# pierluigiferrari/lane_tracker

Hardware: AMD Instinct MI355X
Metric: frames/sec at 1280x720 (end-to-end hot path: undistort+warp+filter_lane_points+sliding_window_search+fit_poly) (higher is better)
Workload: dtype u8; 1 GPU; BASELINE config 3: batch of 256 synthetic lane-like 1280x720 frames per GPU, HBM-resident; warp+filter_lane_points chain + sliding_window_search (26 levels) + fit_poly; bev=1080x1100, parallelism=frames sharded x1, one process per GPU, collective=none (single process), gathered_records_checked=0, streams_per_gpu=4

## Files before the change

include/lane_tracker_amd.h:

```cpp
#ifndef LANE_TRACKER_AMD_H
#define LANE_TRACKER_AMD_H
#include <stddef.h>
#include <stdint.h>

#ifdef __cplusplus
extern "C" {
#endif
#pragma GCC visibility push(default)

#define LT_ABI_VERSION 5

typedef enum lt_status {
    LT_OK = 0,
    LT_ERR_INVALID = -1,
    LT_ERR_HIP = -2,
    LT_ERR_NOMEM = -3,
    LT_ERR_CAPACITY = -4,
    LT_ERR_STATE = -5
} lt_status;

typedef struct lt_ctx lt_ctx;

typedef struct lt_calib {
    int32_t img_w, img_h;
// ... 128 lines not shown

int  lt_bilateral_adaptive_threshold(lt_ctx* ctx, const uint8_t* img, int h, int w, int ksize, int C,
                                     int mode, int true_value, int false_value, uint8_t* out);
int  lt_filter_lane_points(lt_ctx* ctx, const uint8_t* bev_rgb, int h, int w, const lt_filter_params* p,
                           uint8_t* mask);

int  lt_morph_ellipse(lt_ctx* ctx, const uint8_t* img, int h, int w, int k, int op, int direct, uint8_t* out);

int  lt_fit_poly2(lt_ctx* ctx, const int32_t* ys, const int32_t* xs, int n, int h, int w, double coef[3],
                  int* rank_deficient);

int  lt_overlay_configure(lt_ctx* ctx, const double* Minv );
int  lt_overlay_run(lt_ctx* ctx, int first_slot, int n, const int32_t* left_n, const int32_t* right_n,
                    const int32_t* left_yx, const int32_t* right_yx, double alpha);
int  lt_overlay_run_rows(lt_ctx* ctx, int first_slot, int n, const int32_t* left_n, const int32_t* right_n,
                         const int32_t* left_yx, const int32_t* right_yx, double alpha, const int32_t* rows4);
int  lt_overlay_set_font(lt_ctx* ctx, const uint8_t* atlas, const uint8_t* advance, int first_char, int n_glyphs,
                         int glyph_w, int glyph_h);
int  lt_overlay_text(lt_ctx* ctx, int first_slot, int n, const char* lines, int n_lines, int line_len, int x0, int y0,
                     int step);
int  lt_overlay_rows(lt_ctx* ctx, int* row0, int* row1);
int  lt_present_frame(lt_ctx* ctx, int slot, const int32_t* left_n, const int32_t* right_n, const int32_t* left_yx,
                      const int32_t* right_yx, double alpha, const char* lines, int n_lines, int line_len, int x0, int y0,
                      int step, uint8_t* out, const int32_t* rows4);
int  lt_present_lane_async(lt_ctx* ctx, int slot, const int32_t* left_n, const int32_t* right_n, const int32_t* left_yx,
                           const int32_t* right_yx, double alpha, uint8_t* out, const int32_t* rows4);
int  lt_present_finish(lt_ctx* ctx, int slot, const char* lines, int n_lines, int line_len, int x0, int y0, int step,
                       uint8_t* out, const int32_t* rows4);
int  lt_present_lane_from_fit_async(lt_ctx* ctx, int slot, const double* prev_sum, int count, const double* ploty,
                                    const double* ploty2, int n_rows, double alpha, uint8_t* out, const int32_t* rows4);
int  lt_lane_spans_from_fit(lt_ctx* ctx, const double* fit6, int detected, int fit_flags, const double* prev_sum, int count,
                            const double* ploty, const double* ploty2, int n_rows, int16_t* spans_out);
int  lt_lane_polygon_spans(int warp_h, const int32_t* left_yx, int n_left, const int32_t* right_yx, int n_right,
                           int16_t* spans);
int  lt_poly_points(int warp_w, int warp_h, const double* coeffs, int n, const double* ploty, const double* ploty2, int n_rows,
                    int32_t* left_n, int32_t* right_n, int32_t* left_yx, int32_t* right_yx);
int  lt_frame_tail(int warp_w, int warp_h, const double* in, const double* ploty_v, const double* ploty2_v, int n_rows_v, const double* ploty,
                   const double* ploty2, int n_rows, double* avg6, int32_t* left_n, int32_t* right_n, int32_t* left_yx, int32_t* right_yx,
                   double* out);
int  lt_download_overlay(lt_ctx* ctx, int first_slot, int n, uint8_t* out);
int  lt_download_overlay_async(lt_ctx* ctx, int first_slot, int n, uint8_t* out);
int  lt_download_overlay_rows_async(lt_ctx* ctx, int first_slot, int n, uint8_t* out, const int32_t* rows4);
int  lt_download_overlay_wait(lt_ctx* ctx);
int  lt_set_download_method(lt_ctx* ctx, int method);
int  lt_download_stats(lt_ctx* ctx, double* engine_gbs, int* engine_copies, double* kernel_gbs, int* kernel_copies, int* method);
int  lt_overlay_run_strip(lt_ctx* ctx, int first_slot, int n, const int32_t* left_n, const int32_t* right_n, const int32_t* left_yx,
                          const int32_t* right_yx, double alpha);
int  lt_overlay_run_strip_coeffs(lt_ctx* ctx, int first_slot, int n, const double* coeffs, const uint8_t* draw, const double* ploty,
                                 const double* ploty2, int n_rows, double alpha);
int  lt_strip_download_async(lt_ctx* ctx, int first_slot, int n, uint8_t* out, size_t out_frame_stride, int group);
int  lt_text_blend_host(uint8_t* frames, size_t frame_stride, int n, int img_h, int img_w, const uint8_t* atlas, const uint8_t* advance,
                        int first_char, int n_glyphs, int glyph_w, int glyph_h, const char* lines, int n_lines, int line_len, int x0,
                        int y0, int step);
int  lt_host_text_async_group(int group, uint8_t* dst, size_t dst_stride, const uint8_t* src, size_t src_stride, int n, const int32_t* rows4,
                              int img_h, int img_w, const uint8_t* atlas, const uint8_t* advance, int first_char, int n_glyphs,
                              int glyph_w, int glyph_h, const char* lines, int n_lines, int line_len, int x0, int y0, int step);
int  lt_host_text_now_group(int group, uint8_t* frame, int img_h, int img_w, const uint8_t* atlas, const uint8_t* advance, int first_char,
                            int n_glyphs, int glyph_w, int glyph_h, const char* lines, int n_lines, int line_len, int x0, int y0, int step);
int  lt_host_alloc(size_t bytes, void** out);
int  lt_host_copy_async(void* dst, const void* src, size_t bytes);
int  lt_host_copy2d_async(void* dst, size_t dst_pitch, const void* src, size_t src_pitch, size_t width, size_t height);
int  lt_host_copy_wait(void);
int  lt_host_copy_group_create(int* group);
int  lt_host_copy_group_destroy(int group);
int  lt_host_copy_async_group(int group, void* dst, const void* src, size_t bytes);
int  lt_host_copy2d_async_group(int group, void* dst, size_t dst_pitch, const void* src, size_t src_pitch, size_t width, size_t height);
int  lt_host_copy_wait_group(int group);
int  lt_host_touch_async_group(int group, void* p, size_t bytes);
int  lt_shutdown(void);
int  lt_host_copy_stats(double* busy_seconds, double* copied_bytes, long long* pieces, int* threads);
int  lt_host_memory_stats(size_t* staging_bytes, size_t* queued_pieces, size_t* pending_pieces);
int  lt_host_free(void* p);
int  lt_device_cache_trim(size_t keep_bytes);
int  lt_device_cache_stats(size_t* kept_bytes, size_t* live_bytes, size_t* limit_bytes, int* kept_blocks);
int  lt_device_cache_counters(unsigned long long* hits, unsigned long long* misses, unsigned long long* evicted_blocks,
                              unsigned long long* evicted_bytes);
int  lt_download_bev(lt_ctx* ctx, int first_slot, int n, uint8_t* out);

int  lt_calib_source_rows(const lt_calib* calib, int* row0, int* row1);
int  lt_calib_warp_table(const lt_calib* calib, int16_t* xy, uint16_t* frac);
int  lt_calib_undistort_table(const lt_calib* calib, int row0, int row1, int16_t* xy, uint16_t* frac);
int  lt_calib_lab_tables(uint16_t* gamma256, uint16_t* cbrt3072, int32_t* coeffs9);
int  lt_calib_ellipse(int k, int32_t* halfwidths , int* taps);

typedef struct lt_gather lt_gather;
int  lt_gather_init(lt_ctx* ctx, int rank, int world, const char* id_path, int timeout_s, lt_gather** out);
int  lt_gather_world(lt_gather* g, int* rank, int* world);
int  lt_gather_reserve(lt_gather* g, int records_per_rank);
int  lt_gather_stage(lt_gather* g, int first_slot, int n, int at);
int  lt_gather_records(lt_gather* g, int n_records, lt_lane_record* out_host);
int  lt_gather_host(lt_gather* g, const void* in, size_t bytes, void* out);
int  lt_gather_barrier(lt_gather* g);
void lt_gather_destroy(lt_gather* g);

int  lt_timer_start(lt_ctx* ctx);
int  lt_timer_stop(lt_ctx* ctx, float* ms);
int  lt_set_stage_timing(lt_ctx* ctx, int enabled);
int  lt_stage_reset(lt_ctx* ctx);
int  lt_stage_ms(lt_ctx* ctx, float* ms, int32_t* launches, int n);
const char* lt_stage_name(int stage);
#define LT_NO_CONTEXT (-2147483647 - 1)
int  lt_last_threshold_path(lt_ctx* ctx);
int  lt_last_adaptive_path(lt_ctx* ctx);

#pragma GCC visibility pop
#ifdef __cplusplus
}
#endif
#endif
```

lane_tracker_amd/_native.py:

```python
import ctypes as C
import math
import os
import subprocess
import weakref

import numpy as np

_HERE = os.path.dirname(os.path.abspath(__file__))
LIB_PATH = os.environ.get("LANE_TRACKER_AMD_LIB") or os.path.join(_HERE, "liblane_tracker_amd.so")
NUM_STAGES = 12
ABI_VERSION = 5

PLANE_R, PLANE_LAB_B, PLANE_TOPHAT_R, PLANE_TOPHAT_B, PLANE_MERGED, PLANE_MASK = range(6)


class NativeError(RuntimeError):
    pass


class Calib(C.Structure):
    _fields_ = [("img_w", C.c_int32), ("img_h", C.c_int32), ("warp_w", C.c_int32), ("warp_h", C.c_int32),
                ("cam_matrix", C.c_double * 9), ("dist_coeffs", C.c_double * 5), ("M", C.c_double * 9)]


# ... 67 lines not shown
    "lt_download_masks": (C.c_int, [_P, C.c_int, C.c_int, _P]),
    "lt_download_plane": (C.c_int, [_P, C.c_int, C.c_int, C.c_int, _P]),
    "lt_download_undistorted": (C.c_int, [_P, C.c_int, C.c_int, _P]),
    "lt_download_records": (C.c_int, [_P, C.c_int, C.c_int, _P]),
    "lt_download_pixels": (C.c_int, [_P, C.c_int, C.c_int, _P, _P, C.c_int, C.POINTER(C.c_int)]),
    "lt_download_centroids": (C.c_int, [_P, C.c_int, C.c_int, _P, C.c_int, C.POINTER(C.c_int)]),
    "lt_download_lane_lists": (C.c_int, [_P, C.c_int, C.c_void_p, C.c_void_p, C.c_void_p, C.c_void_p, C.c_int, C.POINTER(C.c_int), C.c_int,
                               C.c_void_p, C.c_void_p, C.c_int, C.POINTER(C.c_int)]),
    "lt_copy_records_to_device": (C.c_int, [_P, C.c_int, C.c_int, _P]),
    "lt_enqueue_records_to_device": (C.c_int, [_P, C.c_int, C.c_int, _P]),
    "lt_overlay_configure": (C.c_int, [_P, _P]),
    "lt_overlay_run": (C.c_int, [_P, C.c_int, C.c_int, _P, _P, _P, _P, C.c_double]),
    "lt_overlay_set_font": (C.c_int, [_P, _P, _P, C.c_int, C.c_int, C.c_int, C.c_int]),
    "lt_overlay_text": (C.c_int, [_P, C.c_int, C.c_int, _P, C.c_int, C.c_int, C.c_int, C.c_int, C.c_int]),
    "lt_overlay_rows": (C.c_int, [_P, C.POINTER(C.c_int), C.POINTER(C.c_int)]),
    "lt_present_frame": (C.c_int, [_P, C.c_int, _P, _P, _P, _P, C.c_double, _P, C.c_int, C.c_int, C.c_int, C.c_int, C.c_int, _P, _P]),
    "lt_present_lane_async": (C.c_int, [_P, C.c_int, _P, _P, _P, _P, C.c_double, _P, _P]),
    "lt_present_finish": (C.c_int, [_P, C.c_int, _P, C.c_int, C.c_int, C.c_int, C.c_int, C.c_int, _P, _P]),
    "lt_overlay_run_strip_coeffs": (C.c_int, [_P, C.c_int, C.c_int, _P, _P, _P, _P, C.c_int, C.c_double]),
    "lt_present_lane_from_fit_async": (C.c_int, [_P, C.c_int, _P, C.c_int, _P, _P, C.c_int, C.c_double, _P, _P]),
    "lt_lane_spans_from_fit": (C.c_int, [_P, _P, C.c_int, C.c_int, _P, C.c_int, _P, _P, C.c_int, _P]),
    "lt_lane_polygon_spans": (C.c_int, [C.c_int, _P, C.c_int, _P, C.c_int, _P]),
    "lt_download_overlay": (C.c_int, [_P, C.c_int, C.c_int, _P]),
    "lt_download_overlay_async": (C.c_int, [_P, C.c_int, C.c_int, _P]),
    "lt_download_bev": (C.c_int, [_P, C.c_int, C.c_int, _P]),
    "lt_host_alloc": (C.c_int, [C.c_size_t, C.POINTER(C.c_void_p)]),
    "lt_host_free": (C.c_int, [_P]),
    "lt_host_copy_async": (C.c_int, [_P, _P, C.c_size_t]),
    "lt_host_copy2d_async": (C.c_int, [_P, C.c_size_t, _P, C.c_size_t, C.c_size_t, C.c_size_t]),
    "lt_overlay_run_rows": (C.c_int, [_P, C.c_int, C.c_int, _P, _P, _P, _P, C.c_double, _P]),
    "lt_download_overlay_rows_async": (C.c_int, [_P, C.c_int, C.c_int, _P, _P]),
    "lt_host_copy_wait": (C.c_int, []),
    "lt_host_copy_group_create": (C.c_int, [C.POINTER(C.c_int)]),
    "lt_host_copy_group_destroy": (C.c_int, [C.c_int]),
    "lt_host_copy_async_group": (C.c_int, [C.c_int, _P, _P, C.c_size_t]),
    "lt_host_copy2d_async_group": (C.c_int, [C.c_int, _P, C.c_size_t, _P, C.c_size_t, C.c_size_t, C.c_size_t]),
    "lt_host_copy_wait_group": (C.c_int, [C.c_int]),
    "lt_host_touch_async_group": (C.c_int, [C.c_int, _P, C.c_size_t]),
    "lt_shutdown": (C.c_int, []),
    "lt_host_copy_stats": (C.c_int, [C.POINTER(C.c_double), C.POINTER(C.c_double), C.POINTER(C.c_longlong), C.POINTER(C.c_int)]),
    "lt_warm": (C.c_int, [_P, C.POINTER(SearchParams), C.POINTER(SearchParams), C.c_int]),
    "lt_overlay_run_strip": (C.c_int, [_P, C.c_int, C.c_int, _P, _P, _P, _P, C.c_double]),
    "lt_strip_download_async": (C.c_int, [_P, C.c_int, C.c_int, _P, C.c_size_t, C.c_int]),
    "lt_text_blend_host": (C.c_int, [_P, C.c_size_t, C.c_int, C.c_int, C.c_int, _P, _P, C.c_int, C.c_int, C.c_int, C.c_int, _P, C.c_int,
                                     C.c_int, C.c_int, C.c_int, C.c_int]),
    "lt_host_text_async_group": (C.c_int, [C.c_int, _P, C.c_size_t, _P, C.c_size_t, C.c_int, _P, C.c_int, C.c_int, _P, _P,
                                           C.c_int, C.c_int, C.c_int, C.c_int, _P, C.c_int, C.c_int, C.c_int, C.c_int, C.c_int]),
    "lt_host_text_now_group": (C.c_int, [C.c_int, _P, C.c_int, C.c_int, _P, _P, C.c_int, C.c_int, C.c_int, C.c_int, _P, C.c_int, C.c_int,
                                         C.c_int, C.c_int, C.c_int]),
    "lt_mask_run": (C.c_int, [_P, C.c_int, C.c_int, C.POINTER(FilterParams)]),
    "lt_mask_rerun": (C.c_int, [_P, C.c_int, C.c_int, C.POINTER(FilterParams)]),
    "lt_upload_bev": (C.c_int, [_P, _P, C.c_int, C.c_int]),
    "lt_filter_run": (C.c_int, [_P, C.c_int, C.c_int, C.POINTER(FilterParams)]),
    "lt_sws_fit_run": (C.c_int, [_P, C.c_int, C.c_int, C.POINTER(SearchParams)]),
    "lt_band_fit_run": (C.c_int, [_P, C.c_int, C.c_int, C.POINTER(SearchParams), _P]),
    "lt_search_fit_list": (C.c_int, [_P, C.c_int, _P, C.POINTER(SearchParams), C.POINTER(SearchParams)]),
    "lt_upload_frame_rows_list": (C.c_int, [_P, _P, C.c_int, C.c_int]),
    "lt_upload_frame_rest_list": (C.c_int, [_P, _P, C.c_int, C.c_int]),
    "lt_band_fit_chain_run": (C.c_int, [_P, C.c_int, C.c_int, C.POINTER(SearchParams), _P]),
    "lt_band_fit_chain_collect": (C.c_int, [_P, C.c_int, C.c_int, _P]),
    "lt_band_fit_chain_cancel": (C.c_int, [_P]),
    "lt_set_search_cus": (C.c_int, [_P, C.c_int]),
    "lt_set_walk_min_frames": (C.c_int, [_P, C.c_int]),
    "lt_set_direct_upload": (C.c_int, [_P, C.c_int]),
    "lt_direct_upload_count": (C.c_ulonglong, [_P]),
    "lt_set_urgent": (C.c_int, [_P, C.c_int]),
    "lt_poly_points": (C.c_int, [C.c_int, C.c_int, _P, C.c_int, _P, _P, C.c_int, _P, _P, _P, _P]),
    "lt_frame_tail": (C.c_int, [C.c_int, C.c_int, _P, _P, _P, C.c_int, _P, _P, C.c_int, _P, _P, _P, _P, _P, _P]),
    "lt_download_overlay_wait": (C.c_int, [_P]),
    "lt_set_frame_base": (C.c_int, [_P, C.c_int, C.c_int, C.c_int]),
    "lt_mask_batch": (C.c_int, [_P, _P, C.c_int, C.POINTER(FilterParams), _P]),
    "lt_sws_fit_batch": (C.c_int, [_P, _P, C.c_int, C.POINTER(SearchParams), _P]),
    "lt_band_fit_batch": (C.c_int, [_P, _P, C.c_int, C.POINTER(SearchParams), _P, _P]),
    "lt_bilateral_adaptive_threshold": (C.c_int, [_P, _P, C.c_int, C.c_int, C.c_int, C.c_int, C.c_int, C.c_int,
                                                 C.c_int, _P]),
    "lt_filter_lane_points": (C.c_int, [_P, _P, C.c_int, C.c_int, C.POINTER(FilterParams), _P]),
    "lt_morph_ellipse": (C.c_int, [_P, _P, C.c_int, C.c_int, C.c_int, C.c_int, C.c_int, _P]),
    "lt_fit_poly2": (C.c_int, [_P, _P, _P, C.c_int, C.c_int, C.c_int, C.POINTER(C.c_double), C.POINTER(C.c_int)]),
    "lt_calib_source_rows": (C.c_int, [C.POINTER(Calib), C.POINTER(C.c_int), C.POINTER(C.c_int)]),
    "lt_calib_warp_table": (C.c_int, [C.POINTER(Calib), _P, _P]),
    "lt_calib_undistort_table": (C.c_int, [C.POINTER(Calib), C.c_int, C.c_int, _P, _P]),
    "lt_calib_lab_tables": (C.c_int, [_P, _P, _P]),
    "lt_calib_ellipse": (C.c_int, [C.c_int, _P, C.POINTER(C.c_int)]),
    "lt_gather_init": (C.c_int, [_P, C.c_int, C.c_int, C.c_char_p, C.c_int, C.POINTER(_P)]),
    "lt_gather_world": (C.c_int, [_P, C.POINTER(C.c_int), C.POINTER(C.c_int)]),
    "lt_gather_reserve": (C.c_int, [_P, C.c_int]),
    "lt_gather_stage": (C.c_int, [_P, C.c_int, C.c_int, C.c_int]),
    "lt_gather_records": (C.c_int, [_P, C.c_int, _P]),
    "lt_gather_host": (C.c_int, [_P, _P, C.c_size_t, _P]),
    "lt_gather_barrier": (C.c_int, [_P]),
    "lt_gather_destroy": (None, [_P]),
    "lt_timer_start": (C.c_int, [_P]),
    "lt_timer_stop": (C.c_int, [_P, C.POINTER(C.c_float)]),
    "lt_set_stage_timing": (C.c_int, [_P, C.c_int]),
    "lt_stage_reset": (C.c_int, [_P]),
    "lt_stage_ms": (C.c_int, [_P, C.POINTER(C.c_float), C.POINTER(C.c_int32), C.c_int]),
    "lt_stage_name": (C.c_char_p, [C.c_int]),
    "lt_device_cache_trim": (C.c_int, [C.c_size_t]),
    "lt_device_cache_stats": (C.c_int, [C.POINTER(C.c_size_t), C.POINTER(C.c_size_t), C.POINTER(C.c_size_t), C.POINTER(C.c_int)]),
    "lt_device_cache_counters": (C.c_int, [C.POINTER(C.c_ulonglong)] * 4),
    "lt_host_memory_stats": (C.c_int, [C.POINTER(C.c_size_t)] * 3),
    "lt_set_download_method": (C.c_int, [_P, C.c_int]),
    "lt_download_stats": (C.c_int, [_P, _P, _P, _P, _P, _P]),
    "lt_last_threshold_path": (C.c_int, [_P]),
    "lt_last_adaptive_path": (C.c_int, [_P]),
    "lt_set_input_format": (C.c_int, [_P, C.c_int, _P]),
    "lt_get_input_format": (C.c_int, [_P, C.POINTER(C.c_int), _P]),
    "lt_yuv_to_rgb": (C.c_int, [_P, _P, C.c_int, C.c_int, C.c_int, _P, _P]),
    "lt_attach_device_frames": (C.c_int, [_P, _P, C.c_int, C.c_int]),
    "lt_device_frames_rest": (C.c_int, [_P, C.c_int, C.c_int, _P]),
    "lt_device_alloc": (C.c_int, [C.c_int, C.c_size_t, C.POINTER(C.c_void_p)]),
    "lt_device_free": (C.c_int, [_P]),
    "lt_device_write": (C.c_int, [_P, _P, C.c_size_t]),
    "lt_device_read": (C.c_int, [_P, _P, C.c_size_t]),
    "lt_device_stream_wait": (C.c_int, [C.c_int, C.c_size_t]),
}

PIXEL_FORMATS = {"rgb": 0, "nv12": 1, "i420": 2}
YUV_MATRICES = {"bt601": (1220542, 1673527, -852492, -409993, 2116026),
                "bt709": (1220542, 1880097, -558891, -223347, 2214593)}


def pixel_format_id(pixel_format):
    try:
        return PIXEL_FORMATS[pixel_format]
    except (KeyError, TypeError):
        raise ValueError("pixel_format must be 'rgb', 'nv12' or 'i420', got %r" % (pixel_format,)) from None


def yuv_coeffs(matrix):
    if isinstance(matrix, str):
        if matrix not in YUV_MATRICES:
            raise ValueError("yuv_matrix must be 'bt601' or 'bt709', got %r" % (matrix,))
        matrix = YUV_MATRICES[matrix]
    k = np.ascontiguousarray(matrix, dtype=np.int32)
    if k.shape != (5,):
        raise ValueError("a conversion matrix is five integers")
    return k


def frame_shape(img_size, pixel_format="rgb"):
    w, h = int(img_size[0]), int(img_size[1])
    if pixel_format_id(pixel_format) == 0:
        return (h, w, 3)
    if w % 2 or h % 2:
        raise ValueError("4:2:0 frames need an even width and height, got %dx%d" % (w, h))
    return (h * 3 // 2, w)

_lib = None


def build(force=False):
    csrc = os.path.join(_HERE, "csrc")
    cmd = ["make", "-C", csrc, "-s", "-j8"] + (["-B"] if force else [])
    subprocess.check_call(cmd)
    return LIB_PATH


def load():
    global _lib
    if _lib is not None:
        return _lib
    if not os.path.exists(LIB_PATH):
        raise NativeError(f"{LIB_PATH} is missing: build it with `python -c 'import __graft_entry__ as g; g.build()'` "
                          "(hipcc --offload-arch=gfx950).  lane_tracker_amd has no CPU fallback.")
    lib = C.CDLL(LIB_PATH)
# ... 196 lines not shown
    if rc:
        _check(rc)


def host_copy_stats():
    b, y, p, t = C.c_double(), C.c_double(), C.c_longlong(), C.c_int()
    _check(load().lt_host_copy_stats(C.byref(b), C.byref(y), C.byref(p), C.byref(t)))
    return {"busy_s": b.value, "bytes": y.value, "pieces": p.value, "threads": t.value}


def device_cache_stats():
    k, l, m, n = C.c_size_t(), C.c_size_t(), C.c_size_t(), C.c_int()
    _check(load().lt_device_cache_stats(C.byref(k), C.byref(l), C.byref(m), C.byref(n)))
    return {"kept_bytes": k.value, "live_bytes": l.value, "limit_bytes": m.value, "kept_blocks": n.value}


def host_memory_stats():
    v = [C.c_size_t() for _ in range(3)]
    _check(load().lt_host_memory_stats(*[C.byref(x) for x in v]))
    return dict(zip(("staging_bytes", "queued_pieces", "pending_pieces"), (int(x.value) for x in v)))


def device_cache_counters():
    v = [C.c_ulonglong() for _ in range(4)]
    _check(load().lt_device_cache_counters(*[C.byref(x) for x in v]))
    return dict(zip(("hits", "misses", "evicted_blocks", "evicted_bytes"), (int(x.value) for x in v)))


def pinned_empty(shape, dtype=np.uint8):
    return _pinned.empty(shape, dtype)


def _u8(a, shape_tail=None):
    a = np.ascontiguousarray(a, dtype=np.uint8)
    return a


def filter_params(filter_type="bilateral", ksize_r=15, C_r=8, ksize_b=35, C_b=5, mask_noise=False,
                  noise_thresh=140, ksize_noise=65, C_noise=10):
    ft = {"bilateral": 0, "neighborhood": 1}.get(filter_type, 2)
    return FilterParams(ft, int(ksize_r), int(C_r), int(ksize_b), int(C_b), int(bool(mask_noise)),
                        int(noise_thresh), int(ksize_noise), int(C_noise))


def search_params(window_width=30, window_height=40, search_range=20, mu=0.1, no_success_limit=8,
                  start_slice=0.25, ignore_sides=360, ignore_bottom=30, bandwidth=25, partial=1.0):
    return SearchParams(int(window_width), int(window_height), int(search_range), int(no_success_limit),
                        int(ignore_sides), int(ignore_bottom), int(bandwidth), 0, float(mu), float(start_slice),
                        float(partial))


def make_calib(img_size, warped_size, cam_matrix, dist_coeffs, M):
    cal = Calib()
    cal.img_w, cal.img_h = int(img_size[0]), int(img_size[1])
    cal.warp_w, cal.warp_h = int(warped_size[0]), int(warped_size[1])
    cal.cam_matrix[:] = [float(v) for v in np.asarray(cam_matrix, np.float64).reshape(9)]
    d = np.asarray(dist_coeffs, np.float64).reshape(-1)
    cal.dist_coeffs[:] = [float(v) for v in (list(d[:5]) + [0.0] * 5)[:5]]
    cal.M[:] = [float(v) for v in np.asarray(M, np.float64).reshape(9)]
    return cal


def calib_tables(cal):
    lib = load()
    r0, r1 = C.c_int(0), C.c_int(0)
    _check(lib.lt_calib_source_rows(C.byref(cal), C.byref(r0), C.byref(r1)))
    wxy = np.empty((cal.warp_h, cal.warp_w, 2), np.int16)
    wfr = np.empty((cal.warp_h, cal.warp_w), np.uint16)
    _check(lib.lt_calib_warp_table(C.byref(cal), wxy.ctypes.data, wfr.ctypes.data))
    uxy = np.empty((r1.value - r0.value, cal.img_w, 2), np.int16)
    ufr = np.empty((r1.value - r0.value, cal.img_w), np.uint16)
    _check(lib.lt_calib_undistort_table(C.byref(cal), r0.value, r1.value, uxy.ctypes.data, ufr.ctypes.data))
    gamma, cbrt, coef = np.empty(256, np.uint16), np.empty(3072, np.uint16), np.empty(9, np.int32)
    _check(lib.lt_calib_lab_tables(gamma.ctypes.data, cbrt.ctypes.data, coef.ctypes.data))
    ell = {}
    for k in (5, 29, 55):
        dx, taps = np.empty(k, np.int32), C.c_int(0)
        _check(lib.lt_calib_ellipse(k, dx.ctypes.data, C.byref(taps)))
        ell[k] = (dx, taps.value)
    return dict(source_rows=(r0.value, r1.value), warp_xy=wxy, warp_frac=wfr, und_xy=uxy, und_frac=ufr, gamma=gamma,
                cbrt=cbrt, lab_coeffs=coef, ellipse=ell)


def pack_polygons(polygons):
    ln = np.array([len(p[0]) for p in polygons], np.int32)
    rn = np.array([len(p[2]) for p in polygons], np.int32)

    def pairs(ys, xs, counts):
        out = np.empty((int(counts.sum()), 2), np.int32)
        at = 0
        for y, x, m in zip(ys, xs, counts):
            out[at:at + m, 0] = y
            out[at:at + m, 1] = x
            at += m
        return out
    return ln, rn, pairs([p[0] for p in polygons], [p[1] for p in polygons], ln), pairs([p[2] for p in polygons], [p[3] for p in polygons], rn)


def poly_points(warped_size, coeffs, ploty, ploty2):
    lib = load()
    coeffs = np.ascontiguousarray(coeffs, np.float64).reshape(-1, 6)
    ploty, ploty2 = np.ascontiguousarray(ploty, np.float64), np.ascontiguousarray(ploty2, np.float64)
    n, rows = coeffs.shape[0], ploty.shape[0]
    ln, rn = np.empty(n, np.int32), np.empty(n, np.int32)
    lyx, ryx = np.empty((n * rows, 2), np.int32), np.empty((n * rows, 2), np.int32)
    _check(lib.lt_poly_points(int(warped_size[0]), int(warped_size[1]), coeffs.ctypes.data, n, ploty.ctypes.data, ploty2.ctypes.data,
                              rows, ln.ctypes.data, rn.ctypes.data, lyx.ctypes.data, ryx.ctypes.data))
    return ln, rn, lyx[:int(ln.sum())], ryx[:int(rn.sum())]


class Context:

    def __init__(self, img_size, warped_size, cam_matrix, dist_coeffs, M, device=0, capacity=1):
        self._h = None
        lib = load()
        cal = make_calib(img_size, warped_size, cam_matrix, dist_coeffs, M)
        h = _P()
        _check(lib.lt_create(C.byref(cal), int(device), C.byref(h)))
        self._h = h
        self.lib = lib
        self.img_w, self.img_h, self.warp_w, self.warp_h = cal.img_w, cal.img_h, cal.warp_w, cal.warp_h
        self._frame_tail = (cal.img_h, cal.img_w, 3)
        self.reserve(capacity)

    def close(self):
        if self._h is not None:
            self.lib.lt_destroy(self._h)
            self._h = None

    def __del__(self):
        try:
            self.close()
        except Exception:
            pass

    def reserve(self, capacity):
        _check(self.lib.lt_reserve(self._h, int(capacity)))
        self.capacity = max(getattr(self, "capacity", 0), int(capacity))

    def info(self):
        i = Info()
        _check(self.lib.lt_get_info(self._h, C.byref(i)))
        return i

    def sync(self):
        _check(self.lib.lt_sync(self._h))

    def set_streams(self, n):
        _check(self.lib.lt_set_streams(self._h, int(n)))

    def set_input_format(self, pixel_format="rgb", yuv_matrix="bt601"):
        layout = pixel_format_id(pixel_format)
        tail = frame_shape((self.img_w, self.img_h), pixel_format)
        k = yuv_coeffs(yuv_matrix) if layout else None
        _check(self.lib.lt_set_input_format(self._h, layout, None if k is None else k.ctypes.data))
        self._frame_tail = tail

    def input_format(self):
        layout, k = C.c_int(0), np.zeros(5, np.int32)
        _check(self.lib.lt_get_input_format(self._h, C.byref(layout), k.ctypes.data))
        return {v: n for n, v in PIXEL_FORMATS.items()}[layout.value], tuple(int(v) for v in k)

    def _frames(self, frames):
        f = _u8(frames)
        tail = self._frame_tail
        if f.shape[-len(tail):] != tail or f.ndim > len(tail) + 1:
# ... 496 lines not shown
```

lane_tracker_amd/csrc/k_tophat.hip:

```cpp
#include <cstdlib>

#include <cstdio>
#include <cstdlib>

#include <type_traits>

#include "lt_internal.h"

#ifndef LT_DPP_SELECT
#define LT_DPP_SELECT 0
#endif
#ifndef LT_FUSED55
#define LT_FUSED55 1
#endif

namespace lt {
namespace {

typedef unsigned short u16x2 __attribute__((ext_vector_type(2)));

template <bool DIL>
__device__ __forceinline__ uint32_t pk(uint32_t a, uint32_t b) {
    const u16x2 x = __builtin_bit_cast(u16x2, a), y = __builtin_bit_cast(u16x2, b);
    const u16x2 r = DIL ? __builtin_elementwise_max(x, y) : __builtin_elementwise_min(x, y);
// ... 16 lines not shown
    static constexpr int slot_width[17] = {0, 7, 10, 12, 14, 16, 17, 18, 19, 20, 21, 22, 23, 24, 25, 26, 27};
    static constexpr int slot(int j) { return half_slot[j <= R ? j : K - 1 - j]; }

    template <bool DIL>
    static __device__ __forceinline__ void row_windows(uint32_t* s, int lane, uint32_t (&H)[NH]) {
        uint32_t* S0 = s + MARGIN;
        uint32_t* S1 = S0 + PLANE;
        uint32_t* S2 = S0 + 2 * PLANE;
        uint32_t* S4 = S0 + 3 * PLANE;
        uint32_t* S7 = S0 + 4 * PLANE;
        uint32_t* S14 = S0 + 5 * PLANE;
        const int pa = lane, pb = lane + 64;
        S1[pa] = pk<DIL>(pk<DIL>(S0[pa - 1], S0[pa + 1]), S0[pa]);
        S1[pb] = pk<DIL>(pk<DIL>(S0[pb - 1], S0[pb + 1]), S0[pb]);
        wave_lds_fence();
        S2[pa] = pk<DIL>(S1[pa - 1], S1[pa + 1]);
        S2[pb] = pk<DIL>(S1[pb - 1], S1[pb + 1]);
        wave_lds_fence();
        S4[pa] = pk<DIL>(S2[pa - 2], S2[pa + 2]);
        S4[pb] = pk<DIL>(S2[pb - 2], S2[pb + 2]);
        wave_lds_fence();
        S7[pa] = pk<DIL>(S4[pa - 3], S4[pa + 3]);
        S7[pb] = pk<DIL>(S4[pb - 3], S4[pb + 3]);
        wave_lds_fence();
        S14[pa] = pk<DIL>(S7[pa - 7], S7[pa + 7]);
        S14[pb] = pk<DIL>(S7[pb - 7], S7[pb + 7]);
        wave_lds_fence();
        const int p = R + lane;
        H[0] = S0[p];
        H[1] = S7[p];
        H[2] = pk<DIL>(S7[p - 3], S7[p + 3]);
        H[3] = pk<DIL>(S7[p - 5], S7[p + 5]);
        H[4] = S14[p];
#pragma unroll
        for (int t = 2; t <= 13; ++t) H[3 + t] = pk<DIL>(S14[p - t], S14[p + t]);
    }
};

struct SE29 {
    static constexpr int K = 29, R = 14, NH = 9, NPLANES = 5;
    static constexpr int half_slot[15] = {0, 1, 2, 3, 4, 5, 5, 6, 7, 7, 7, 8, 8, 8, 8};
    static constexpr int slot_width[9] = {0, 5, 7, 9, 10, 11, 12, 13, 14};
    static constexpr int slot(int j) { return half_slot[j <= R ? j : K - 1 - j]; }

    template <bool DIL>
    static __device__ __forceinline__ void row_windows(uint32_t* s, int lane, uint32_t (&H)[NH]) {
        uint32_t* S0 = s + MARGIN;
        uint32_t* S1 = S0 + PLANE;
        uint32_t* S2 = S0 + 2 * PLANE;
        uint32_t* S4 = S0 + 3 * PLANE;
        uint32_t* S7 = S0 + 4 * PLANE;
        const int pa = lane, pb = lane + 64;
        S1[pa] = pk<DIL>(pk<DIL>(S0[pa - 1], S0[pa + 1]), S0[pa]);
        S1[pb] = pk<DIL>(pk<DIL>(S0[pb - 1], S0[pb + 1]), S0[pb]);
        wave_lds_fence();
        S2[pa] = pk<DIL>(S1[pa - 1], S1[pa + 1]);
        S2[pb] = pk<DIL>(S1[pb - 1], S1[pb + 1]);
        wave_lds_fence();
        S4[pa] = pk<DIL>(S2[pa - 2], S2[pa + 2]);
        S4[pb] = pk<DIL>(S2[pb - 2], S2[pb + 2]);
        wave_lds_fence();
        S7[pa] = pk<DIL>(S4[pa - 3], S4[pa + 3]);
        S7[pb] = pk<DIL>(S4[pb - 3], S4[pb + 3]);
        wave_lds_fence();
        const int p = R + lane;
        H[0] = S0[p];
        H[1] = pk<DIL>(S4[p - 1], S4[p + 1]);
        H[2] = S7[p];
#pragma unroll
        for (int t = 2; t <= 7; ++t) H[1 + t] = pk<DIL>(S7[p - t], S7[p + t]);
    }
};

struct RunsGeom {
    int h, w, nstrips, nbands, band_rows, ntasks;
    size_t plane_stride;
    int dpitch;
    size_t dst_stride;
    int nframes;
    int nstrips_normal;
    int n_normal;
    int xcd;
    uint8_t* copy_dst;
};

struct LaneCols {
    uint32_t off[4];
    uint32_t keep[2];
    uint32_t fill[2];
};

__device__ __forceinline__ LaneCols lane_cols(int col0, int w, bool second, uint32_t n8) {
    LaneCols c;
#pragma unroll
    for (int e = 0; e < 2; ++e) {
        const int ca = col0 + 64 * e, cb = ca + 64;
        const bool va = ca >= 0 && ca < w && (e == 0 || second), vb = cb >= 0 && cb < w && (e == 0 || second);
        c.off[2 * e] = (uint32_t)min(max(ca, 0), w - 1);
        c.off[2 * e + 1] = (uint32_t)min(max(cb, 0), w - 1);
        c.keep[e] = (va ? 0xffffu : 0u) | (vb ? 0xffff0000u : 0u);
        c.fill[e] = (va ? 0u : n8) | (vb ? 0u : (n8 << 16));
    }
    return c;
}

__device__ __forceinline__ uint32_t fetch_entry(const uint8_t* __restrict__ row, const LaneCols& c, int e) {
    const uint32_t a = row[c.off[2 * e]], b = row[c.off[2 * e + 1]];
    return ((a | (b << 16)) & c.keep[e]) | c.fill[e];
}

__device__ __forceinline__ uint32_t fetch_entry(__amdgpu_buffer_rsrc_t plane, int row_off, const LaneCols& c, int e) {
    const uint32_t a = __builtin_amdgcn_raw_buffer_load_b8(plane, (int)c.off[2 * e], row_off, 0);
    const uint32_t b = __builtin_amdgcn_raw_buffer_load_b8(plane, (int)c.off[2 * e + 1], row_off, 0);
    return ((a | (b << 16)) & c.keep[e]) | c.fill[e];
}

template <class SE, bool DIL>
__global__ __launch_bounds__(256) void k_morph_runs(const uint8_t* __restrict__ src, uint8_t* __restrict__ dst,
                                                   const uint8_t* __restrict__ minuend, RunsGeom g) {
    __shared__ uint32_t s_chain[4][SE::NPLANES * PLANE];
    constexpr int K = SE::K, R = SE::R, NH = SE::NH;
    constexpr uint32_t NEUTRAL = DIL ? 0u : 0x00ff00ffu;
    const int lane = threadIdx.x & 63, wv = threadIdx.x >> 6;
    const int task = __builtin_amdgcn_readfirstlane(blockIdx.x * 4 + wv);
    if (task >= g.ntasks) return;
    const int strip = task % g.nstrips;
    const int band = (task / g.nstrips) % g.nbands;
    const int frame = task / (g.nstrips * g.nbands);
    const uint8_t* s = src + (size_t)frame * g.plane_stride;
    uint8_t* d = dst + (size_t)frame * g.dst_stride;
    const uint8_t* m = minuend ? minuend + (size_t)frame * g.plane_stride : nullptr;
    uint32_t* chain = s_chain[wv];
    const int x0 = strip * 128;
    const int yb0 = band * g.band_rows, yb1 = min(yb0 + g.band_rows, g.h);
    const int xa = x0 + lane, xb = xa + 64;
    const bool va = xa < g.w, vb = xb < g.w;
    const int oa = min(xa, g.w - 1), ob = min(xb, g.w - 1);

    uint32_t A[K];
#pragma unroll
    for (int j = 0; j < K; ++j) A[j] = NEUTRAL;

    const int y_first = yb0 - R, y_last = yb1 - 1 + R;
    const LaneCols cols = lane_cols(x0 - R + lane, g.w, lane + 64 < 64 + 2 * R, NEUTRAL & 0xffu);
    const uint8_t* row = s + (size_t)min(max(y_first, 0), g.h - 1) * g.w;
    uint32_t e0 = fetch_entry(row, cols, 0), e1 = fetch_entry(row, cols, 1);
    uint32_t ma = 0, mb = 0;
    for (int yy = y_first; yy <= y_last; ++yy) {
        const bool in_img = yy >= 0 && yy < g.h;
        chain[MARGIN + lane] = in_img ? e0 : NEUTRAL;
        chain[MARGIN + lane + 64] = in_img ? e1 : NEUTRAL;
        wave_lds_fence();
        row = s + (size_t)min(max(yy + 1, 0), g.h - 1) * g.w;
        e0 = fetch_entry(row, cols, 0);
        e1 = fetch_entry(row, cols, 1);
        const int y = yy - R;
        const uint32_t ma_cur = ma, mb_cur = mb;
        if (m) {
            const uint8_t* mrow = m + (size_t)min(max(y + 1, 0), g.h - 1) * g.w;
            ma = mrow[oa];
            mb = mrow[ob];
        }

        uint32_t H[NH];
        SE::template row_windows<DIL>(chain, lane, H);
        wave_lds_fence();
// ... 188 lines not shown
            updates(std::integral_constant<int, 4>{});
        }
        asm volatile("s_waitcnt lgkmcnt(0)" : "+v"(a5), "+v"(b5), "+v"(c5), "+v"(d5), "+v"(e5) :: "memory");
        {
            LT_PAIR(15, a5, b5)
            Ha[16] = op3<DIL>(lo(c5), lo(d5), lo(e5)); Hb[16] = op3<DIL>(hi(c5), hi(d5), hi(e5));
            updates(std::integral_constant<int, 5>{});
        }
#undef LT_WAIT8
#undef LT_PAIR
#undef LT_G
#pragma unroll
        for (int j = 0; j < K; ++j) A[j] = An[j];
        out_ab[1] = A[0];
    } else if (SE::K == 55) {
        LT_STEP3(2, 3, 9)
        const uint32_t a4 = lds_addr(S4 + p - 8), a13 = lds_addr(SL + p - 14);
        unsigned long long r0, f[7], g[29];
        LT_RD64(r0, s0_rd, 0);
        LT_RD64(f[0], a4, 0);
        LT_RD64(f[1], a4, 16);
        LT_RD64(f[2], a4, 40);
        LT_RD64(f[3], a4, 64);
        LT_RD64(f[4], a4, 88);
        LT_RD64(f[5], a4, 112);
        LT_RD64(f[6], a4, 128);
#define LT_G(i) LT_RD64(g[i], a13, (i) * 8)
        LT_G(0); LT_G(1); LT_G(2); LT_G(3); LT_G(4); LT_G(5); LT_G(6); LT_G(7); LT_G(8); LT_G(9); LT_G(10); LT_G(11);
        LT_G(13); LT_G(14); LT_G(15);
        LT_G(17); LT_G(18); LT_G(19); LT_G(20); LT_G(21); LT_G(22); LT_G(23); LT_G(24); LT_G(25); LT_G(26); LT_G(27); LT_G(28);
#undef LT_G
        asm volatile("s_waitcnt lgkmcnt(0)"
                     : "+v"(r0), "+v"(f[0]), "+v"(f[1]), "+v"(f[2]), "+v"(f[3]), "+v"(f[4]), "+v"(f[5]), "+v"(f[6]),
                       "+v"(g[0]), "+v"(g[1]), "+v"(g[2]), "+v"(g[3]), "+v"(g[4]), "+v"(g[5]), "+v"(g[6]), "+v"(g[7]),
                       "+v"(g[8]), "+v"(g[9]), "+v"(g[10]), "+v"(g[11]), "+v"(g[13]), "+v"(g[14]), "+v"(g[15])
                     :: "memory");
        asm volatile("" : "+v"(g[17]), "+v"(g[18]), "+v"(g[19]), "+v"(g[20]), "+v"(g[21]), "+v"(g[22]), "+v"(g[23]),
                          "+v"(g[24]), "+v"(g[25]), "+v"(g[26]), "+v"(g[27]), "+v"(g[28]) :: "memory");
        __builtin_amdgcn_sched_barrier(0);
        Ha[0] = lo(r0); Hb[0] = hi(r0);
        Ha[1] = op2<DIL>(lo(f[2]), lo(f[4])); Hb[1] = op2<DIL>(hi(f[2]), hi(f[4]));
        Ha[2] = op3<DIL>(lo(f[1]), lo(f[3]), lo(f[5])); Hb[2] = op3<DIL>(hi(f[1]), hi(f[3]), hi(f[5]));
        Ha[3] = op3<DIL>(lo(f[0]), lo(f[3]), lo(f[6])); Hb[3] = op3<DIL>(hi(f[0]), hi(f[3]), hi(f[6]));
        Ha[4] = op2<DIL>(lo(g[13]), lo(g[15])); Hb[4] = op2<DIL>(hi(g[13]), hi(g[15]));
#pragma unroll
        for (int q = 3; q <= 13; ++q) {
            Ha[2 + q] = op2<DIL>(lo(g[14 - q]), lo(g[14 + q]));
            Hb[2 + q] = op2<DIL>(hi(g[14 - q]), hi(g[14 + q]));
        }
        Ha[16] = op3<DIL>(lo(g[0]), lo(g[14]), lo(g[28])); Hb[16] = op3<DIL>(hi(g[0]), hi(g[14]), hi(g[28]));
    } else {
        const uint32_t a4 = lds_addr(S4 + p - 10);
        unsigned long long r0, g[21];
        LT_PRIO_READS2();
        LT_RD64(r0, s0_rd, 0);
#define LT_G(i) LT_RD64(g[i], a4, (i) * 8)
        LT_G(9); LT_G(11); LT_G(7); LT_G(13); LT_G(10); LT_G(5); LT_G(15); LT_G(4); LT_G(16); LT_G(3); LT_G(17); LT_G(2); LT_G(18);
        LT_G(1); LT_G(19); LT_G(0); LT_G(20);
#undef LT_G
        LT_PRIO_MATH2();
        asm volatile("s_waitcnt lgkmcnt(10)" : "+v"(r0), "+v"(g[9]), "+v"(g[11]), "+v"(g[7]), "+v"(g[13]), "+v"(g[10]), "+v"(g[5]), "+v"(g[15]) :: "memory");
        Ha[0] = lo(r0); Hb[0] = hi(r0);
        Ha[1] = op2<DIL>(lo(g[9]), lo(g[11])); Hb[1] = op2<DIL>(hi(g[9]), hi(g[11]));
        Ha[2] = op2<DIL>(lo(g[7]), lo(g[13])); Hb[2] = op2<DIL>(hi(g[7]), hi(g[13]));
        Ha[3] = op3<DIL>(lo(g[5]), lo(g[10]), lo(g[15])); Hb[3] = op3<DIL>(hi(g[5]), hi(g[10]), hi(g[15]));
        asm volatile("" : "+v"(Ha[0]), "+v"(Hb[0]), "+v"(Ha[1]), "+v"(Hb[1]), "+v"(Ha[2]), "+v"(Hb[2]), "+v"(Ha[3]), "+v"(Hb[3]));
        asm volatile("s_waitcnt lgkmcnt(0)"
                     : "+v"(g[0]), "+v"(g[1]), "+v"(g[2]), "+v"(g[3]), "+v"(g[4]), "+v"(g[16]), "+v"(g[17]), "+v"(g[18]), "+v"(g[19]), "+v"(g[20])
                     :: "memory");
#pragma unroll
        for (int t = 6; t <= 9; ++t) {
            Ha[t - 2] = op3<DIL>(lo(g[10 - t]), lo(g[10]), lo(g[10 + t]));
            Hb[t - 2] = op3<DIL>(hi(g[10 - t]), hi(g[10]), hi(g[10 + t]));
        }
        Ha[8] = op3<DIL>(Ha[2], lo(g[0]), lo(g[20])); Hb[8] = op3<DIL>(Hb[2], hi(g[0]), hi(g[20]));

    }
#undef LT_STEP3
#undef LT_RD64
}

template <class SE, bool DIL, bool WIDE, bool TH, bool PAIR, bool COPYM = false>
__device__ __forceinline__ void morph_task(const uint8_t* __restrict__ src, uint8_t* __restrict__ dst, const uint8_t* __restrict__ minuend,
                                           const RunsGeom& g, uint2* chain, uint8_t* s_out_w, int lane, int strip, int band, int frame) {
    static_assert(WIDE || !PAIR, "pair strips exist for the WIDE kernels only");
    static_assert(!COPYM || (WIDE && TH), "the minuend copy rides on the dword store of the WIDE top-hat");
    constexpr int K = SE::K, R = SE::R, NH = SE::NH;
    constexpr uint32_t NEUTRAL = (DIL ? 0u : 0x00ff00ffu) | BIAS2;
    const uint8_t* s = src + (size_t)frame * g.plane_stride;
    uint8_t* d = dst + (size_t)frame * g.dst_stride;
    const uint8_t* m = TH ? minuend + (size_t)frame * g.plane_stride : nullptr;
    const bool has_b = PAIR && frame + 1 < g.nframes;
    const bool lane_b = PAIR && (lane & 16);
    const int x0 = strip * 128;
    const int yb0 = band * g.band_rows, yb1 = min(yb0 + g.band_rows, g.h);
    const int xa = x0 + lane, xb = xa + 64;
    const bool va = xa < g.w, vb = xb < g.w;
    const int oa = min(xa, g.w - 1), ob = min(xb, g.w - 1);

    const int wcol = x0 + 4 * (lane & (PAIR ? 15 : 31)), wcol_c = min(wcol, g.w - 4);
    const uint32_t row_sel = lane < 32 ? 0x06040200u : 0x07050301u;

    uint32_t A[K];
#pragma unroll
    for (int j = 0; j < K; ++j) A[j] = NEUTRAL;

    const int y_first = yb0 - R, y_last = yb1 - 1 + R;
    const int c0 = x0 - R + lane;
    const uint32_t col_a = (uint32_t)min(max(c0, 0), g.w - 1), col_b = (uint32_t)min(max(c0 + 64, 0), g.w - 1), col_c = (uint32_t)min(max(c0 + 128, 0), g.w - 1);
    constexpr int RSRC_RAW = 0x00027000;
    const int plane_bytes = g.h * g.w;
    const int b_src = has_b ? (int)g.plane_stride : 0;
    const __amdgpu_buffer_rsrc_t src_rs = __builtin_amdgcn_make_buffer_rsrc(const_cast<uint8_t*>(s), 0, plane_bytes + b_src, RSRC_RAW);
    const __amdgpu_buffer_rsrc_t dst_rs = __builtin_amdgcn_make_buffer_rsrc(d + (size_t)yb0 * g.dpitch, 0, (yb1 - yb0) * g.dpitch + (has_b ? (int)g.dst_stride : 0), RSRC_RAW);
    const __amdgpu_buffer_rsrc_t min_rs = __builtin_amdgcn_make_buffer_rsrc(const_cast<uint8_t*>(TH ? m : s), 0, plane_bytes + b_src, RSRC_RAW);
    const __amdgpu_buffer_rsrc_t cp_rs = __builtin_amdgcn_make_buffer_rsrc(
        (COPYM ? g.copy_dst + (size_t)frame * g.dst_stride : d) + (size_t)yb0 * g.dpitch, 0, (yb1 - yb0) * g.dpitch + (has_b ? (int)g.dst_stride : 0), RSRC_RAW);
    auto row_ptr = [&](int y) { return __mul24(min(max(y, 0), g.h - 1), g.w); };
    struct Raw { uint32_t a, b, c, d; };
    const uint32_t sel_ab = 0x0c000c00u | ((4u + (col_b & 3u)) << 16) | (col_a & 3u);
    const uint32_t sel_bc = 0x0c000c00u | ((4u + (col_c & 3u)) << 16) | (col_b & 3u);
    const uint32_t sel_pa = 0x0c000c00u | ((4u + (col_a & 3u)) << 16) | (col_a & 3u);
    const uint32_t sel_pb = 0x0c000c00u | ((4u + (col_b & 3u)) << 16) | (col_b & 3u);
    auto load_row = [&](int y) __attribute__((always_inline)) {
        const int ro = row_ptr(y);
        Raw r;
        r.d = 0;
        if (PAIR) {
            r.a = __builtin_amdgcn_raw_buffer_load_b32(src_rs, (int)(col_a & ~3u), ro, 0);
            r.b = __builtin_amdgcn_raw_buffer_load_b32(src_rs, (int)(col_b & ~3u), ro, 0);
            r.c = __builtin_amdgcn_raw_buffer_load_b32(src_rs, (int)(col_a & ~3u), ro + b_src, 0);
            r.d = __builtin_amdgcn_raw_buffer_load_b32(src_rs, (int)(col_b & ~3u), ro + b_src, 0);
        } else if (WIDE) {
            r.a = __builtin_amdgcn_raw_buffer_load_b32(src_rs, (int)(col_a & ~3u), ro, 0);
            r.b = __builtin_amdgcn_raw_buffer_load_b32(src_rs, (int)(col_b & ~3u), ro, 0);
            r.c = __builtin_amdgcn_raw_buffer_load_b32(src_rs, (int)(col_c & ~3u), ro, 0);
        } else {
            r.a = __builtin_amdgcn_raw_buffer_load_b8(src_rs, (int)col_a, ro, 0);
            r.b = __builtin_amdgcn_raw_buffer_load_b8(src_rs, (int)col_b, ro, 0);
            r.c = __builtin_amdgcn_raw_buffer_load_b8(src_rs, (int)col_c, ro, 0);
        }
        return r;
    };
    auto combine = [&](const Raw& r, uint32_t& e0, uint32_t& e1) __attribute__((always_inline)) {
        if (PAIR) {
            asm volatile("v_perm_b32 %0, %4, %2, %6\n\tv_perm_b32 %1, %5, %3, %7" : "=&v"(e0), "=&v"(e1) : "v"(r.a), "v"(r.b), "v"(r.c), "v"(r.d), "v"(sel_pa), "v"(sel_pb));
        } else if (WIDE) {
            asm volatile("v_perm_b32 %0, %3, %2, %5\n\tv_perm_b32 %1, %4, %3, %6" : "=&v"(e0), "=&v"(e1) : "v"(r.a), "v"(r.b), "v"(r.c), "v"(sel_ab), "v"(sel_bc));
        } else {
            e0 = r.a | (r.b << 16);
            e1 = r.b | (r.c << 16);
            asm volatile("" : "+v"(e0), "+v"(e1));
        }
        if (LT_MORPH_BIAS) { e0 |= BIAS2; e1 |= BIAS2; }
    };
    uint32_t ea0, ea1, eb0, eb1;
    combine(load_row(y_first), ea0, ea1);
    combine(load_row(y_first + 1), eb0, eb1);
    uint32_t ma0 = 0, mb0 = 0, ma1 = 0, mb1 = 0;
    uint32_t m_off = (uint32_t)(__mul24(yb0 - 2 * R + (lane >> 5), g.w) + wcol_c + (lane_b ? b_src : 0));
    uint32_t st_off = wcol < g.w && (!lane_b || has_b) ? (uint32_t)(__mul24(-2 * R - 2 + (lane >> 5), g.dpitch) + wcol + (lane_b ? (int)g.dst_stride : 0))
                                                      : 0x80000000u;
    uint32_t mcur = 0;
    const uint32_t s0_rd = (uint32_t)(uintptr_t)(chain + MARGIN + ((R + lane) & 63));
    const uint32_t out_wr = (uint32_t)(uintptr_t)(s_out_w + (WIDE ? 2 * lane : 0));
    const uint32_t out_rd = (uint32_t)(uintptr_t)(s_out_w + (WIDE ? 8 * (lane & 31) : 0));
    auto out_issue = [&](unsigned long long& q) { asm volatile("ds_read_b64 %0, %1" : "=v"(q) : "v"(out_rd) : "memory"); };
    auto out_finish = [&](unsigned long long q, uint32_t mp, int yp) {
        asm volatile("s_waitcnt lgkmcnt(0)" : "+v"(q) :: "memory");
        uint32_t v = __builtin_amdgcn_perm((uint32_t)(q >> 32), (uint32_t)q, row_sel);
        if (TH) v = mp - v;
        if (PAIR) {
            const int row = yp + (lane >> 5);
            if (row >= yb0 && row < yb1) {
                __builtin_amdgcn_raw_buffer_store_b32(v, dst_rs, (int)st_off, 0, 0);
                if (COPYM) __builtin_amdgcn_raw_buffer_store_b32(mp, cp_rs, (int)st_off, 0, 0);
            }
        } else {
            __builtin_amdgcn_raw_buffer_store_b32(v, dst_rs, (int)st_off, 0, 0);
            if (COPYM) __builtin_amdgcn_raw_buffer_store_b32(mp, cp_rs, (int)st_off, 0, 0);
        }
    };
    auto row_pair = [&](int yy) __attribute__((always_inline)) {
        const uint2 e_pa = make_uint2(ea0, eb0);
        const uint2 e_pb = make_uint2(ea1, eb1);
        chain[MARGIN + lane] = lane < R ? e_pb : e_pa;
        wave_lds_fence();
        const Raw ra = load_row(yy + 2), rb = load_row(yy + 3);
        const int y = yy - R;
        const uint32_t ca0 = ma0, cb0 = mb0, ca1 = ma1, cb1 = mb1;
        const uint32_t mprev = mcur;
        if (TH) {
            if (WIDE) {
                mcur = __builtin_amdgcn_raw_buffer_load_b32(min_rs, (int)m_off, 0, 0);
            } else {
                const uint8_t* r0 = m + (size_t)min(max(y + 2, 0), g.h - 1) * g.w;
                const uint8_t* r1 = m + (size_t)min(max(y + 3, 0), g.h - 1) * g.w;
                ma0 = r0[oa]; mb0 = r0[ob];
                ma1 = r1[oa]; mb1 = r1[ob];
            }
        }
        uint32_t Ha[NH], Hb[NH];
        constexpr bool FUSE = LT_FUSED55 && K == 55;
        uint32_t out_ab[2];
        row_windows2<SE, DIL, FUSE>(chain, lane, e_pa, e_pb, s0_rd, Ha, Hb, A, out_ab);
        wave_lds_fence();
        const bool prev_out = WIDE && y - 1 >= yb0 && y - 2 < yb1;
        unsigned long long q = 0;
        if (prev_out) out_issue(q);
        if (WIDE) __builtin_amdgcn_sched_barrier(0);
        if (!FUSE) {
            out_ab[0] = op2<DIL>(A[1], Ha[SE::slot(0)]);
#pragma unroll
            for (int j = 0; j < K - 2; ++j) A[j] = op3<DIL>(A[j + 2], Ha[SE::slot(j + 1)], Hb[SE::slot(j)]);
            A[K - 2] = op2<DIL>(Ha[SE::slot(K - 1)], Hb[SE::slot(K - 2)]);
            A[K - 1] = Hb[SE::slot(K - 1)];
            out_ab[1] = A[0];
        }
        const uint32_t out_a = out_ab[0], out_b = out_ab[1];
        if (WIDE) {
            __builtin_amdgcn_sched_barrier(0);
            out_finish(q, mprev, y - 2);
            if (y + 1 >= yb0 && y < yb1) {
                const uint32_t W = __builtin_amdgcn_perm(out_b, out_a, 0x06020400u);
                asm volatile("ds_write_b16 %0, %1\n\tds_write_b16_d16_hi %0, %1 offset:128" :: "v"(out_wr), "v"(W) : "memory");
            }
            m_off += 2u * (uint32_t)g.w;
            st_off += 2u * (uint32_t)g.dpitch;
        } else
#pragma unroll
        for (int rr = 0; rr < 2; ++rr) {
            const int yo = y + rr;
            if (yo >= yb0 && yo < yb1) {
                const uint32_t o2 = rr == 0 ? out_a : out_b;
                uint32_t oa_v = o2 & 0xffu, ob_v = (o2 >> 16) & 0xffu;
                if (TH) {
                    const uint32_t qa = rr == 0 ? ca0 : ca1, qb = rr == 0 ? cb0 : cb1;
                    oa_v = qa - oa_v;
                    ob_v = qb - ob_v;
                }
                const size_t o = (size_t)yo * g.dpitch;
                if (va) d[o + xa] = (uint8_t)oa_v;
                if (vb) d[o + xb] = (uint8_t)ob_v;
            }
        }
        combine(ra, ea0, ea1);
        combine(rb, eb0, eb1);
    };
    constexpr int PAIRS = (LT_FUSED55 && K == 55) ? 2 : 1;
    for (int yy = y_first; yy <= y_last; yy += 2 * PAIRS) {
        row_pair(yy);
        if (PAIRS == 2) row_pair(yy + 2);
    }
    if (WIDE) {
        const int npairs = (y_last - y_first) / 2 + 1, pairs_run = (npairs + PAIRS - 1) / PAIRS * PAIRS;
        const int y_tail = y_first + 2 * (pairs_run - 1) - R;
        unsigned long long q;
        out_issue(q);
        out_finish(q, mcur, y_tail);
    }
}

#ifndef LT_MORPH_WPB
#define LT_MORPH_WPB 4
#endif
#ifdef LT_MORPH_MAX_WAVES
#define LT_MORPH_WAVES_ATTR __attribute__((amdgpu_waves_per_eu(1, LT_MORPH_MAX_WAVES)))
#else
#define LT_MORPH_WAVES_ATTR
#endif
template <class SE, bool DIL, bool WIDE, bool TH, bool COPYM = false>
__global__ __launch_bounds__(64 * LT_MORPH_WPB) LT_MORPH_WAVES_ATTR void k_morph_runs2(const uint8_t* __restrict__ src, uint8_t* __restrict__ dst,
                                                    const uint8_t* __restrict__ minuend, RunsGeom g) {
    __shared__ uint2 s_chain[LT_MORPH_WPB][4 * PLANE];
    __shared__ __attribute__((aligned(8))) uint8_t s_out[WIDE ? LT_MORPH_WPB : 1][WIDE ? 256 : 8];
    const int lane = threadIdx.x & 63, wv = threadIdx.x >> 6;
    uint32_t bid = blockIdx.x;
    if (g.xcd) {
        const uint32_t total = gridDim.x, q = total >> 3, r = total & 7u, xcd = bid & 7u, k = bid >> 3;
        bid = (xcd < r ? xcd * (q + 1) : r * (q + 1) + (xcd - r) * q) + k;
    }
    const int task = __builtin_amdgcn_readfirstlane((int)bid * LT_MORPH_WPB + wv);
    if (task >= g.ntasks) return;
    if (!LT_MORPH_BIAS) __builtin_amdgcn_s_setreg(1 | (6 << 6) | (1 << 11), 3);
    const int n_pair = g.ntasks - g.n_normal;
    if (!WIDE || task >= n_pair) {
        const int t = task - n_pair;
        const int strip = t % g.nstrips_normal;
        const int band = (t / g.nstrips_normal) % g.nbands;
        const int frame = t / (g.nstrips_normal * g.nbands);
        morph_task<SE, DIL, WIDE, TH, false, COPYM>(src, dst, minuend, g, s_chain[wv], s_out[wv], lane, strip, band, frame);
    } else if constexpr (WIDE) {
        morph_task<SE, DIL, WIDE, TH, true, COPYM>(src, dst, minuend, g, s_chain[wv], s_out[wv], lane, g.nstrips_normal, task % g.nbands, 2 * (task / g.nbands));
    }
}

template <class SE, bool DIL, bool TH, int Q>
__device__ __forceinline__ void morph_one_task(const int task, const uint8_t* __restrict__ src, uint8_t* __restrict__ dst,
                                               const uint8_t* __restrict__ minuend, const RunsGeom& g, uint2 (*s_chain)[4 * PLANE],
                                               uint32_t (*s_ring)[3 * 2 * Q][64]) {
    constexpr int K = SE::K, R = SE::R, NH = SE::NH, S = 2 * Q, RING = 3 * S;
    static_assert(S - 1 <= K - 1, "the pipeline must be longer than a step");
    const int lane = threadIdx.x & 63, wv = __builtin_amdgcn_readfirstlane((int)(threadIdx.x >> 6));
    if (!LT_MORPH_BIAS) __builtin_amdgcn_s_setreg(1 | (6 << 6) | (1 << 11), 3);
    const int strip = task % g.nstrips;
    const int band = (task / g.nstrips) % g.nbands;
    const int frame = task / (g.nstrips * g.nbands);
    const uint8_t* s = src + (size_t)frame * g.plane_stride;
    uint8_t* d = dst + (size_t)frame * g.dst_stride;
    const uint8_t* m = TH ? minuend + (size_t)frame * g.plane_stride : nullptr;
    uint2* chain = s_chain[wv];
    const int x0 = strip * 128;
    const int yb0 = band * g.band_rows, yb1 = min(yb0 + g.band_rows, g.h);
    const int xa = x0 + lane, xb = xa + 64;
    const bool va = xa < g.w, vb = xb < g.w;
    const int oa = min(xa, g.w - 1), ob = min(xb, g.w - 1);
    const int y_first = yb0 - R, y_base = yb0 - 2 * R;
    const int npairs = (yb1 - yb0 + 2 * R + 1) / 2, nsteps = (npairs + Q - 1) / Q;
    const int c0 = x0 - R + lane;
    const uint32_t col_a = (uint32_t)min(max(c0, 0), g.w - 1), col_b = (uint32_t)min(max(c0 + 64, 0), g.w - 1), col_c = (uint32_t)min(max(c0 + 128, 0), g.w - 1);
    constexpr int RSRC_RAW = 0x00027000;
    const __amdgpu_buffer_rsrc_t src_rs = __builtin_amdgcn_make_buffer_rsrc(const_cast<uint8_t*>(s), 0, g.h * g.w, RSRC_RAW);
    auto row_off = [&](int y) { return __mul24(min(max(y, 0), g.h - 1), g.w); };
    const uint32_t sel_ab = 0x0c000c00u | ((4u + (col_b & 3u)) << 16) | (col_a & 3u);
    const uint32_t sel_bc = 0x0c000c00u | ((4u + (col_c & 3u)) << 16) | (col_b & 3u);
    struct Raw { uint32_t a, b, c; };
    auto load_row = [&](int y) __attribute__((always_inline)) {
        const int ro = row_off(y);
        Raw r;
        r.a = __builtin_amdgcn_raw_buffer_load_b32(src_rs, (int)(col_a & ~3u), ro, 0);
        r.b = __builtin_amdgcn_raw_buffer_load_b32(src_rs, (int)(col_b & ~3u), ro, 0);
        r.c = __builtin_amdgcn_raw_buffer_load_b32(src_rs, (int)(col_c & ~3u), ro, 0);
        return r;
    };
    auto combine = [&](const Raw& r, uint32_t& e0, uint32_t& e1) __attribute__((always_inline)) {
        asm volatile("v_perm_b32 %0, %3, %2, %5\n\tv_perm_b32 %1, %4, %3, %6" : "=&v"(e0), "=&v"(e1) : "v"(r.a), "v"(r.b), "v"(r.c), "v"(sel_ab), "v"(sel_bc));
        if (LT_MORPH_BIAS) { e0 |= BIAS2; e1 |= BIAS2; }
    };
    constexpr uint32_t NEUTRAL = (DIL ? 0u : 0x00ff00ffu) | BIAS2;
    uint32_t A[K + 1];
#pragma unroll
    for (int p = 0; p <= K; ++p) A[p] = NEUTRAL;
    uint32_t ea0, ea1, eb0, eb1;
    {
        const int yy = y_first + 2 * wv;
        combine(load_row(yy), ea0, ea1);
        combine(load_row(yy + 1), eb0, eb1);
    }
    const uint32_t s0_rd = (uint32_t)(uintptr_t)(chain + MARGIN + ((R + lane) & 63));
    for (int t = 0; t < nsteps; ++t) {
        const int yy = y_first + 2 * (t * Q + wv);
        const uint2 e_pa = make_uint2(ea0, eb0);
        const uint2 e_pb = make_uint2(ea1, eb1);
        chain[MARGIN + lane] = lane < R ? e_pb : e_pa;
        wave_lds_fence();
        const Raw ra = load_row(yy + S), rb = load_row(yy + S + 1);
        const int o0 = S * t + 2 * wv, yo = y_base + o0;
        uint32_t m0a = 0, m0b = 0, m1a = 0, m1b = 0;
        if (TH) {
            const uint8_t* r0 = m + (size_t)min(max(yo, 0), g.h - 1) * g.w;
            const uint8_t* r1 = m + (size_t)min(max(yo + 1, 0), g.h - 1) * g.w;
            m0a = r0[oa]; m0b = r0[ob];
            m1a = r1[oa]; m1b = r1[ob];
        }
        uint32_t Ha[NH], Hb[NH];
        row_windows2<SE, DIL, false>(chain, lane, e_pa, e_pb, s0_rd, Ha, Hb);
        wave_lds_fence();
        uint32_t An[K + 1];
#pragma unroll
        for (int p = 0; p <= K; ++p) {
            const int j = p - 1;
            const bool prev = j + S <= K - 1, ha = j <= K - 2, hb = j >= 0;
            const uint32_t va_ = Ha[SE::slot(j + 1 <= K - 1 ? j + 1 : K - 1)], vb_ = Hb[SE::slot(j >= 0 ? j : 0)];
            const uint32_t vp = A[prev ? p + S : K];
            An[p] = prev && ha && hb ? op3<DIL>(vp, va_, vb_) : prev && ha ? op2<DIL>(vp, va_) : ha && hb ? op2<DIL>(va_, vb_) : vb_;
        }
// ... 8 lines not shown
#pragma unroll
        for (int p = S; p <= K; ++p) A[p] = An[p];
        __syncthreads();
        {
            const int sl0 = o0 % RING, sl1 = sl0 + 1 == RING ? 0 : sl0 + 1;
            uint32_t v0 = s_ring[0][sl0][lane], v1 = s_ring[0][sl1][lane];
#pragma unroll
            for (int q = 1; q < Q; ++q) {
                v0 = op2<DIL>(v0, s_ring[q][sl0][lane]);
                v1 = op2<DIL>(v1, s_ring[q][sl1][lane]);
            }
#pragma unroll
            for (int rr = 0; rr < 2; ++rr) {
                const int y = yo + rr;
                if (y >= yb0 && y < yb1) {
                    const uint32_t v = rr == 0 ? v0 : v1;
                    uint32_t pa = v & 0xffu, pb = (v >> 16) & 0xffu;
                    if (TH) {
                        pa = (rr == 0 ? m0a : m1a) - pa;
                        pb = (rr == 0 ? m0b : m1b) - pb;
                    }
                    const size_t o = (size_t)y * g.dpitch;
                    if (va) d[o + xa] = (uint8_t)pa;
                    if (vb) d[o + xb] = (uint8_t)pb;
                }
            }
        }
        combine(ra, ea0, ea1);
        combine(rb, eb0, eb1);
    }
}

template <class SE, bool DIL, bool TH, int Q>
__global__ __launch_bounds__(64 * Q) void k_morph_one(const uint8_t* __restrict__ src, uint8_t* __restrict__ dst,
                                                      const uint8_t* __restrict__ minuend, RunsGeom g) {
    __shared__ uint2 s_chain[Q][4 * PLANE];
    __shared__ uint32_t s_ring[Q][3 * 2 * Q][64];
    morph_one_task<SE, DIL, TH, Q>((int)blockIdx.x, src, dst, minuend, g, s_chain, s_ring);
}

template <bool DIL, bool TH, int Q>
__global__ __launch_bounds__(64 * Q) void k_morph_one_pair(const uint8_t* __restrict__ src55, uint8_t* __restrict__ dst55, const uint8_t* __restrict__ min55, RunsGeom g55,
                                                           const uint8_t* __restrict__ src29, uint8_t* __restrict__ dst29, const uint8_t* __restrict__ min29, RunsGeom g29) {
    __shared__ uint2 s_chain[Q][4 * PLANE];
    __shared__ uint32_t s_ring[Q][3 * 2 * Q][64];
    const int task = (int)blockIdx.x;
    if (task < g55.ntasks) morph_one_task<SE55, DIL, TH, Q>(task, src55, dst55, min55, g55, s_chain, s_ring);
    else morph_one_task<SE29, DIL, TH, Q>(task - g55.ntasks, src29, dst29, min29, g29, s_chain, s_ring);
}

template <class SE, int Q>
void launch_one(hipStream_t s, const uint8_t* src, uint8_t* dst, const uint8_t* minuend, bool dilate, const RunsGeom& g) {
    const dim3 grid(g.ntasks), block(64 * Q);
    if (dilate && minuend) hipLaunchKernelGGL((k_morph_one<SE, true, true, Q>), grid, block, 0, s, src, dst, minuend, g);
    else if (dilate) hipLaunchKernelGGL((k_morph_one<SE, true, false, Q>), grid, block, 0, s, src, dst, minuend, g);
    else hipLaunchKernelGGL((k_morph_one<SE, false, false, Q>), grid, block, 0, s, src, dst, minuend, g);
}

static void one_frame_bands(RunsGeom& g, int n, int want_wgs) {
    int cus1 = 256, dev1 = 0;
    (void)hipGetDevice(&dev1);
    (void)hipDeviceGetAttribute(&cus1, hipDeviceAttributeMultiprocessorCount, dev1);
    const int target = want_wgs > 0 ? want_wgs : 2 * cus1;
    int nb = std::max(1, target / std::max(1, n * g.nstrips));
    int rows = std::max((g.h + nb - 1) / nb, 8);
    rows = (rows + 1) & ~1;
    g.band_rows = rows;
    g.nbands = (g.h + rows - 1) / rows;
    g.nstrips_normal = g.nstrips;
    g.ntasks = g.n_normal = n * g.nstrips * g.nbands;
    g.xcd = 0;
}

template <class SE>
bool table_matches(const EllipseSE& se) {
    if (se.k != SE::K) return false;
    for (int j = 0; j < SE::K; ++j)
        if (SE::slot_width[SE::slot(j)] != se.dx[j]) return false;
    return true;
}

template <class SE>
bool launch_runs(hipStream_t s, const uint8_t* src, uint8_t* dst, const uint8_t* minuend, int h, int w, bool dilate,
                 size_t plane_stride, int n, int dpitch, size_t dst_stride, uint8_t* copy_dst) {
    RunsGeom g;
    g.copy_dst = copy_dst;
    g.h = h;
    g.w = w;
    g.plane_stride = plane_stride;
    g.dpitch = dpitch > 0 ? dpitch : w;
    g.dst_stride = dpitch > 0 ? dst_stride : plane_stride;
    g.nstrips = (w + 127) / 128;
    g.nframes = n;
    static const bool one_row = [] { const char* e = LT_EXP_ENV("LT_MORPH_ONE_ROW"); return e && e[0] == '1'; }();
    static const bool narrow = [] { const char* e = LT_EXP_ENV("LT_MORPH_WIDE"); return e && e[0] == '0'; }();
    const bool wide = !narrow && (w & 3) == 0 && (plane_stride & 3) == 0 && w >= 4 && (g.dpitch & 3) == 0 && (g.dst_stride & 3) == 0 &&
                      ((uintptr_t)dst & 3) == 0 && ((uintptr_t)minuend & 3) == 0;
    static const int one_q = [] { const char* e = LT_EXP_ENV("LT_MORPH_ONE"); return e ? std::atoi(e) : 4; }();
    if (n <= 2 && (one_q == 4 || one_q == 8) && !one_row && wide && !copy_dst && ((uintptr_t)src & 3) == 0) {
        static const int want_wgs = [] { const char* e = LT_EXP_ENV("LT_MORPH_ONE_WGS"); return e ? std::atoi(e) : 0; }();
        one_frame_bands(g, n, want_wgs);
        if (one_q == 8) launch_one<SE, 8>(s, src, dst, minuend, dilate, g);
        else launch_one<SE, 4>(s, src, dst, minuend, dilate, g);
        return true;
    }
    int dev = 0, cus = 256, blocks_per_cu = 3;
    (void)hipGetDevice(&dev);
    (void)hipDeviceGetAttribute(&cus, hipDeviceAttributeMultiprocessorCount, dev);
    {
        const void* fn = one_row ? (dilate ? (const void*)k_morph_runs<SE, true> : (const void*)k_morph_runs<SE, false>)
                                 : wide ? (dilate ? (minuend ? (const void*)k_morph_runs2<SE, true, true, true> : (const void*)k_morph_runs2<SE, true, true, false>)
                                                  : (const void*)k_morph_runs2<SE, false, true, false>)
                                        : (dilate ? (minuend ? (const void*)k_morph_runs2<SE, true, false, true> : (const void*)k_morph_runs2<SE, true, false, false>)
                                                  : (const void*)k_morph_runs2<SE, false, false, false>);
        int nb = 0;
        const int threads = one_row ? 256 : 64 * LT_MORPH_WPB;
        if (hipOccupancyMaxActiveBlocksPerMultiprocessor(&nb, fn, threads, 0) == hipSuccess && nb > 0) blocks_per_cu = nb * threads / 256;
        if (blocks_per_cu < 1) blocks_per_cu = 1;
    }
    const long long slots = (long long)cus * blocks_per_cu * 4, simds = (long long)cus * 4;
    int best_nb = 1;
    double best_cost = 1e300;
    for (int nb = 1; nb <= 256; ++nb) {
        const int rows = (h + nb - 1) / nb;
        const int real_nb = (h + rows - 1) / rows;
        const long long tasks = (long long)n * g.nstrips * real_nb;
        if (nb > 1 && rows < (tasks <= simds ? 4 : tasks <= slots ? (SE::R + 1) / 2 : 2 * SE::R)) break;
        const double rounds = (double)((tasks + slots - 1) / slots);
        const double cost = tasks <= simds ? (double)(rows + 2 * SE::R) : tasks < slots ? 1.15 * (rows + 2 * SE::R) : rounds * (rows + 2 * SE::R);
        if (cost < best_cost - 1e-9) { best_cost = cost; best_nb = nb; }
    }
    if ((long long)n * g.nstrips * 4 >= slots && h / 4 >= 2 * SE::R) best_nb = 4;
    else if ((long long)n * g.nstrips * 4 >= slots / 4 && h / 4 >= 2 * SE::R) best_nb = 4;
#ifdef LT_EXPERIMENTS
    {
        char name[32];
        std::snprintf(name, sizeof name, "LT_MORPH_NB_%d%c", SE::K, dilate ? 'D' : 'E');
        const char* e = std::getenv(name);
        if (e && std::atoi(e) > 0) best_nb = std::atoi(e);
    }
#endif
    g.band_rows = (h + best_nb - 1) / best_nb;
    g.nbands = (h + g.band_rows - 1) / g.band_rows;
    static const bool no_pair = [] { const char* e = LT_EXP_ENV("LT_MORPH_PAIR"); return e && e[0] == '0'; }();
    const bool pair_strip = wide && !one_row && !no_pair && w - 128 * (g.nstrips - 1) <= 64 &&
                            (long long)plane_stride + (long long)h * w < (1ll << 31) && (long long)g.dst_stride + (long long)h * g.dpitch < (1ll << 31);
    g.nstrips_normal = pair_strip ? g.nstrips - 1 : g.nstrips;
    g.n_normal = n * g.nstrips_normal * g.nbands;
    g.ntasks = g.n_normal + (pair_strip ? (n + 1) / 2 * g.nbands : 0);
    static const bool want_xcd = [] { const char* e = LT_EXP_ENV("LT_MORPH_XCD"); return e && e[0] == '1'; }();
    g.xcd = want_xcd ? 1 : 0;
    dim3 grid((g.ntasks + 3) / 4);
    const dim3 grid2((g.ntasks + LT_MORPH_WPB - 1) / LT_MORPH_WPB), block2(64 * LT_MORPH_WPB);
    if (copy_dst && one_row) return false;
    if (one_row) {
        if (dilate) hipLaunchKernelGGL((k_morph_runs<SE, true>), grid, dim3(256), 0, s, src, dst, minuend, g);
        else hipLaunchKernelGGL((k_morph_runs<SE, false>), grid, dim3(256), 0, s, src, dst, minuend, g);
    } else {
        static const int extra_lds = [] { const char* e = LT_EXP_ENV("LT_MORPH_EXTRA_LDS"); return e ? std::atoi(e) : 0; }();
        const bool th = dilate && minuend != nullptr;
        if (copy_dst) {
            if constexpr (SE::K == 55) {
                if (!wide || !th || ((uintptr_t)copy_dst & 3)) return false;
                hipLaunchKernelGGL((k_morph_runs2<SE, true, true, true, true>), grid2, block2, extra_lds, s, src, dst, minuend, g);
                return true;
            } else
                return false;
        }
#define LT_LAUNCH(DIL_, WIDE_, TH_) hipLaunchKernelGGL((k_morph_runs2<SE, DIL_, WIDE_, TH_>), grid2, block2, extra_lds, s, src, dst, minuend, g)
        if (wide) {
            if (th) LT_LAUNCH(true, true, true);
            else if (dilate) LT_LAUNCH(true, true, false);
            else LT_LAUNCH(false, true, false);
        } else {
            if (th) LT_LAUNCH(true, false, true);
            else if (dilate) LT_LAUNCH(true, false, false);
            else LT_LAUNCH(false, false, false);
        }
#undef LT_LAUNCH
    }
    return copy_dst == nullptr;
}

}

bool tophat_tables_match(const EllipseSE& se29, const EllipseSE& se55) {
    return table_matches<SE29>(se29) && table_matches<SE55>(se55);
}

bool launch_morph_runs(hipStream_t s, const uint8_t* src, uint8_t* dst, const uint8_t* minuend, int h, int w, int k,
                       bool dilate, size_t plane_stride, int n, int dpitch, size_t dst_stride, uint8_t* copy_dst) {
    if (n <= 0 || h <= 0 || w <= 0) return true;
    if (k == 55)
        return launch_runs<SE55>(s, src, dst, minuend, h, w, dilate, plane_stride, n, dpitch, dst_stride, copy_dst);
    return launch_runs<SE29>(s, src, dst, minuend, h, w, dilate, plane_stride, n, dpitch, dst_stride, copy_dst);
}

bool launch_morph_one_pair(hipStream_t s, const uint8_t* src55, uint8_t* dst55, const uint8_t* min55, const uint8_t* src29, uint8_t* dst29,
                           const uint8_t* min29, int h, int w, bool dilate, size_t plane_stride, int n, int dpitch, size_t dst_stride) {
    if (n <= 0 || n > 2 || h <= 0 || w < 4) return false;
    RunsGeom g;
    g.copy_dst = nullptr;
    g.h = h;
    g.w = w;
    g.plane_stride = plane_stride;
    g.dpitch = dpitch > 0 ? dpitch : w;
    g.dst_stride = dpitch > 0 ? dst_stride : plane_stride;
    g.nstrips = (w + 127) / 128;
    g.nframes = n;
    auto aligned = [](const void* q) { return ((uintptr_t)q & 3) == 0; };
    if ((w & 3) || (plane_stride & 3) || (g.dpitch & 3) || (g.dst_stride & 3) || !aligned(src55) || !aligned(dst55) || !aligned(min55) ||
        !aligned(src29) || !aligned(dst29) || !aligned(min29) || (dilate && (min55 == nullptr) != (min29 == nullptr)))
        return false;
    RunsGeom g55 = g, g29 = g;
    static const int wgs55 = [] { const char* e = LT_EXP_ENV("LT_PAIR_WGS55"); return e ? std::atoi(e) : 0; }();
    static const int wgs29 = [] { const char* e = LT_EXP_ENV("LT_PAIR_WGS29"); return e ? std::atoi(e) : 0; }();
    static const int pair_q = [] { const char* e = LT_EXP_ENV("LT_PAIR_Q"); return e ? std::atoi(e) : 4; }();
    int cus = 256, dev = 0;
    (void)hipGetDevice(&dev);
    (void)hipDeviceGetAttribute(&cus, hipDeviceAttributeMultiprocessorCount, dev);
    one_frame_bands(g55, n, wgs55 > 0 ? wgs55 : cus);
    one_frame_bands(g29, n, wgs29 > 0 ? wgs29 : cus + cus / 2);
    const dim3 grid(g55.ntasks + g29.ntasks);
#define LT_PAIR(Q_)                                                                                                                              \
    do {                                                                                                                                         \
        const dim3 block(64 * Q_);                                                                                                               \
        if (dilate && min55) hipLaunchKernelGGL((k_morph_one_pair<true, true, Q_>), grid, block, 0, s, src55, dst55, min55, g55, src29, dst29, min29, g29);   \
        else if (dilate) hipLaunchKernelGGL((k_morph_one_pair<true, false, Q_>), grid, block, 0, s, src55, dst55, min55, g55, src29, dst29, min29, g29);      \
        else hipLaunchKernelGGL((k_morph_one_pair<false, false, Q_>), grid, block, 0, s, src55, dst55, min55, g55, src29, dst29, min29, g29);                 \
    } while (0)
#ifdef LT_EXPERIMENTS
    if (pair_q == 8) { LT_PAIR(8); return true; }
#endif
    (void)pair_q;
    LT_PAIR(4);
#undef LT_PAIR
    return true;
}

namespace { __global__ void k_preload_k_tophat() {} }
void preload_k_tophat(hipStream_t s) { hipLaunchKernelGGL(k_preload_k_tophat, dim3(1), dim3(1), 0, s); }

}
```

lane_tracker_amd/csrc/lt_api.cpp:

```cpp
#include <algorithm>
#include <atomic>
#include <cmath>
#include <cstdarg>
#include <cstdio>
#include <cstdlib>
#include <chrono>
#include <condition_variable>
#include <cstring>
#include <deque>
#include <map>
#include <memory>
#include <mutex>
#include <string>
#include <thread>
#include <tuple>
#include <vector>
#include <immintrin.h>
#include <sys/mman.h>
#include <unistd.h>

#include <hip/hip_ext.h>

#include "lt_ctx.h"

// ... 255 lines not shown
    preload_k_threshold(s);
    preload_k_threshold_walk(s);
    preload_k_adaptive_walk(s);
    preload_k_search(s);
    preload_k_overlay(s);
    (void)hipStreamSynchronize(s);
    (void)hipGetLastError();
}

int ensure_bev(lt_ctx* c) {
    if (c->d_bev) return LT_OK;
    return dev_alloc(&c->d_bev, (size_t)c->capacity * c->bev_bytes);
}

void mark_masks(lt_ctx* c, int first, int n, int bits_ok, int u8_ok) {
    for (int i = first; i < first + n && i < (int)c->mask_bits_ok.size(); ++i) {
        c->mask_bits_ok[(size_t)i] = (uint8_t)bits_ok;
        c->mask_u8_ok[(size_t)i] = (uint8_t)u8_ok;
    }
}
bool masks_have_bits(const lt_ctx* c, int first, int n) {
    for (int i = first; i < first + n; ++i)
        if (!c->mask_bits_ok[(size_t)i]) return false;
    return true;
}
int ensure_u8_masks(lt_ctx* c, int first, int n) {
    bool any = false;
    for (int i = first; i < first + n; ++i) any = any || !c->mask_u8_ok[(size_t)i];
    int rc = ensure_plane(c, P_MASK);
    if (rc) return rc;
    if (!any) return LT_OK;
    if ((rc = sync_all(c))) return rc;
    for (int i = first; i < first + n;) {
        if (c->mask_u8_ok[(size_t)i]) { ++i; continue; }
        int j = i;
        while (j < first + n && !c->mask_u8_ok[(size_t)j]) ++j;
        launch_bits_to_u8(c->stream, slot_bits(c, i, true).bits, slot_mask(c, i),
                          c->calib.warp_h, c->calib.warp_w, c->plane_bytes, c->bits_stride, j - i);
        for (int k = i; k < j; ++k) c->mask_u8_ok[(size_t)k] = 1;
        i = j;
    }
    HIP_TRY(hipGetLastError());
    HIP_TRY(hipStreamSynchronize(c->stream));
    return LT_OK;
}

int ensure_noise_buffers(lt_ctx* c) {
    if (c->d_b_pad && c->d_bits_n1 && c->d_bits_n2) return LT_OK;
    const size_t n = (size_t)c->capacity;
    int rc;
    if (!c->d_b_pad && (rc = dev_alloc(&c->d_b_pad, n * c->th_pad_bytes))) return rc;
    if (!c->d_bits_n1 && (rc = dev_alloc(&c->d_bits_n1, n * c->bits_stride))) return rc;
    if (!c->d_bits_n2 && (rc = dev_alloc(&c->d_bits_n2, n * c->bits_stride))) return rc;
    return LT_OK;
}

int validate_filter(const lt_filter_params* p) {
    if (!p) return fail(LT_ERR_INVALID, "null filter params");
    if (p->filter_type != 0 && p->filter_type != 1)
        return fail(LT_ERR_INVALID, "Unexpected filter mode. Expected modes are 'bilateral' or 'neighborhood'.");
    if (p->ksize_r < 1 || p->ksize_b < 1 || (p->mask_noise && p->ksize_noise < 1))
        return fail(LT_ERR_INVALID, "filter sizes must be >= 1");
    if (p->filter_type == 1 && ((p->ksize_r & 1) == 0 || (p->ksize_b & 1) == 0))
        return fail(LT_ERR_INVALID, "'neighborhood' block sizes must be odd (cv2.adaptiveThreshold requirement)");
    if (p->ksize_r > 128 || p->ksize_b > 128 || p->ksize_noise > 128)
        return fail(LT_ERR_INVALID, "filter size too large (max 128)");
    return LT_OK;
}

int ensure_plane(lt_ctx* c, int idx) {
    if (c->d_plane[idx]) return LT_OK;
    int rc = dev_alloc(&c->d_plane[idx], (size_t)c->capacity * c->plane_bytes);
    if (rc) return rc;
    if (idx == P_MASK) {
        HIP_TRY(hipMemsetAsync(c->d_plane[idx], 0, (size_t)c->capacity * c->plane_bytes, c->stream));
        HIP_TRY(hipStreamSynchronize(c->stream));
    }
    return LT_OK;
}

constexpr int SIDE_LANES = 10;

int run_filter_chain(lt_ctx* c, hipStream_t s, int first, int n, const lt_filter_params* p, int h, int w, int call_frames,
                     bool u8_mask = false) {
    const size_t ps = c->plane_bytes, off = (size_t)first * ps;
    uint8_t* R = c->d_plane[P_R] + off;
    uint8_t* B = c->d_plane[P_B] + off;
    uint8_t* thR = c->d_plane[P_THR] + off;
    uint8_t* thB = c->d_plane[P_THB] + off;
    uint8_t* t0 = c->d_plane[P_T0] + off;
    uint8_t *t1 = nullptr, *t2 = nullptr, *t3 = nullptr;
    auto scratch = [&](int idx, uint8_t*& q) -> int {
        const int rc = ensure_plane(c, idx);
        if (!rc) q = c->d_plane[idx] + off;
        return rc;
    };
    uint8_t* mask = nullptr;
    if (u8_mask) { const int rc = scratch(P_MASK, mask); if (rc) return rc; }
    const bool walk = p->filter_type == 0 && !c->brute_tophat && c->d_th_pad[0] && c->d_bits_tmp && c->d_bits_tmp2 &&
                      first + n <= (int)c->th_padded.size() && (long long)call_frames * h * w >= c->walk_min_pixels &&
                      bilateral_walk_supported(p->ksize_r, p->C_r, p->ksize_b, p->C_b, h, w, c->th_pitch) &&
                      (!p->mask_noise || noise_walk_supported(p->ksize_noise, p->C_noise, h, w, c->th_pitch));
    const bool walk_noise = walk && p->mask_noise;
    if (walk_noise) {
        const int rc = ensure_noise_buffers(c);
        if (rc) return rc;
    }
    uint8_t* bpad = walk_noise ? c->d_b_pad + (size_t)first * c->th_pad_bytes : nullptr;
    if (p->filter_type == 0) c->last_threshold_path = walk ? 1 : 0;
    const int dpitch = walk ? c->th_pitch : 0;
    uint8_t* thRd = walk ? c->d_th_pad[0] + (size_t)first * c->th_pad_bytes : thR;
    uint8_t* thBd = walk ? c->d_th_pad[1] + (size_t)first * c->th_pad_bytes : thB;
    auto tophat_b = [&](hipStream_t st) -> int {
        if (bpad && launch_morph_runs(st, t0, thBd, B, h, w, 55, true, ps, n, dpitch, c->th_pad_bytes, bpad)) return LT_OK;
        launch_morph_runs(st, t0, thBd, B, h, w, 55, true, ps, n, dpitch, c->th_pad_bytes);
        if (bpad)
            for (int i = 0; i < n; ++i)
                HIP_TRY(hipMemcpy2DAsync(bpad + (size_t)i * c->th_pad_bytes, (size_t)c->th_pitch, B + (size_t)i * ps, (size_t)w, (size_t)w,
                                         (size_t)h, hipMemcpyDeviceToDevice, st));
        return LT_OK;
    };
    if (p->filter_type == 0 && first + n <= (int)c->th_padded.size())
        for (int i = first; i < first + n; ++i) c->th_padded[(size_t)i] = walk ? 1 : 0;
    unsigned long long* mbits = c->d_bits_merged + (size_t)first * c->bits_stride;
    unsigned long long* ebits = c->d_bits_eroded + (size_t)first * c->bits_stride;
    unsigned long long* tbits = c->d_bits_tmp ? c->d_bits_tmp + (size_t)first * c->bits_stride : nullptr;
    unsigned long long* ubits = c->d_bits_tmp2 ? c->d_bits_tmp2 + (size_t)first * c->bits_stride : nullptr;
    bool both_split = false;
    if (p->filter_type == 0) {
        if (c->brute_tophat) {
            { StageScope t(c, ST_ERODE_R, s);  launch_morph_ellipse(s, R, t0, nullptr, h, w, c->se29, false, ps, n); }
            { StageScope t(c, ST_TOPHAT_R, s); launch_morph_ellipse(s, t0, thR, R, h, w, c->se29, true, ps, n); }
            { StageScope t(c, ST_ERODE_B, s);  launch_morph_ellipse(s, B, t0, nullptr, h, w, c->se55, false, ps, n); }
            { StageScope t(c, ST_TOPHAT_B, s); launch_morph_ellipse(s, t0, thB, B, h, w, c->se55, true, ps, n); }
        } else if (n <= 2 && !c->stage_timing && !walk) {
            if (!c->d_side_scratch) { const int rc = dev_alloc(&c->d_side_scratch, (size_t)SIDE_LANES * 2 * ps); if (rc) return rc; }
            int lane_of_stream = SIDE_LANES - 1;
            for (int i = 0; i < (int)c->streams.size() && i < SIDE_LANES - 1; ++i)
                if (c->streams[(size_t)i] == s) { lane_of_stream = i; break; }
            uint8_t* ts = c->d_side_scratch + (size_t)lane_of_stream * 2 * ps;
            if (launch_morph_one_pair(s, B, t0, nullptr, R, ts, nullptr, h, w, false, ps, n, 0, 0)) {
                if (!launch_morph_one_pair(s, t0, thB, B, ts, thR, R, h, w, true, ps, n, 0, 0)) {
                    launch_morph_runs(s, t0, thB, B, h, w, 55, true, ps, n);
                    launch_morph_runs(s, ts, thR, R, h, w, 29, true, ps, n);
                }
            } else {
                launch_morph_runs(s, R, t0, nullptr, h, w, 29, false, ps, n);
                launch_morph_runs(s, t0, thR, R, h, w, 29, true, ps, n);
                launch_morph_runs(s, B, t0, nullptr, h, w, 55, false, ps, n);
                launch_morph_runs(s, t0, thB, B, h, w, 55, true, ps, n);
            }
            both_split = !p->mask_noise;
        } else {
            { StageScope t(c, ST_ERODE_R, s);  launch_morph_runs(s, R, t0, nullptr, h, w, 29, false, ps, n); }
            { StageScope t(c, ST_TOPHAT_R, s); launch_morph_runs(s, t0, thRd, R, h, w, 29, true, ps, n, dpitch, c->th_pad_bytes); }
            { StageScope t(c, ST_ERODE_B, s);  launch_morph_runs(s, B, t0, nullptr, h, w, 55, false, ps, n); }
            { StageScope t(c, ST_TOPHAT_B, s); const int rc = tophat_b(s); if (rc) return rc; }
        }
    }
    bool merged_done = false, partials = false;
    bool two_partials = false;
    unsigned long long *nbits1 = nullptr, *nbits2 = nullptr;
    if (p->filter_type == 0) {
        StageScope t(c, ST_THRESHOLD, s);
        if (walk) {
            merged_done = launch_bilateral_walk(s, thRd, p->ksize_r, p->C_r, thBd, p->ksize_b, p->C_b, mbits, ebits, tbits, ubits,
                                                h, w, c->th_pitch, c->th_pad_bytes, c->bits_stride, n, false) == 0;
            partials = merged_done;
            if (merged_done && walk_noise) {
                nbits1 = c->d_bits_n1 + (size_t)first * c->bits_stride;
                nbits2 = c->d_bits_n2 + (size_t)first * c->bits_stride;
                if (launch_noise_walk(s, bpad, p->ksize_noise, p->C_noise, p->noise_thresh, nbits1, nbits2, h, w, c->th_pitch,
                                      c->th_pad_bytes, c->bits_stride, n))
                    return fail(LT_ERR_STATE, "the greenery-mask walk refused parameters its own predicate accepted");
            }
        }
        if (!merged_done && both_split) {
            merged_done = launch_bilateral_bits(s, thR, p->ksize_r, p->C_r, thB, p->ksize_b, p->C_b, B, p->ksize_noise, p->C_noise,
                                                p->noise_thresh, 0, mbits, h, w, ps, c->bits_stride, n, ebits) == 0;
            partials = two_partials = merged_done;
        }
        if (!merged_done)
          merged_done = launch_bilateral_bits(s, thR, p->ksize_r, p->C_r, thB, p->ksize_b, p->C_b, B, p->ksize_noise,
                                            p->C_noise, p->noise_thresh, p->mask_noise ? 1 : 0, mbits, h, w, ps,
                                            c->bits_stride, n) == 0;
        if (!merged_done) {
            { int rc = scratch(P_T1, t1); if (!rc) rc = scratch(P_T2, t2); if (rc) return rc; }
            launch_bilateral(s, thR, t1, h, w, p->ksize_r, p->C_r, 0, 255, 0, ps, n);
            launch_bilateral(s, thB, t2, h, w, p->ksize_b, p->C_b, 0, 255, 0, ps, n);
        }
    } else {
        StageScope t(c, ST_THRESHOLD, s);
        if (!p->mask_noise && launch_adaptive_walk(s, R, p->ksize_r, p->C_r, mbits, B, p->ksize_b, p->C_b, ebits, h, w, ps, c->bits_stride, n)) {
            merged_done = true;
            partials = true;
            two_partials = true;
        } else {
            { int rc = scratch(P_T1, t1); if (!rc) rc = scratch(P_T2, t2); if (rc) return rc; }
            launch_adaptive_mean(s, R, t1, h, w, p->ksize_r, p->C_r, ps, n);
            launch_adaptive_mean(s, B, t2, h, w, p->ksize_b, p->C_b, ps, n);
        }
        c->last_adaptive_path = two_partials ? 1 : 0;
    }
    if (!merged_done) {
        { const int rc = scratch(P_T3, t3); if (rc) return rc; }
        if (p->mask_noise) {
            StageScope t(c, ST_THRESHOLD, s);
            launch_bilateral(s, B, t3, h, w, p->ksize_noise, p->C_noise, 0, 255, 0, ps, n);
        }
        StageScope t(c, ST_MERGE, s);
        launch_pack_merge(s, t1, t2, B, t3, p->noise_thresh, p->mask_noise ? 1 : 0, mbits, h, w, ps, c->bits_stride, n);
    }
    { StageScope t(c, ST_OPEN, s);
      unsigned long long* obits = c->d_bits_open + (size_t)first * c->bits_stride;
      bool opened = false;
      if (!u8_mask && n >= 16)
          opened = launch_merge_open5(s, mbits, partials ? ebits : nullptr, two_partials ? nullptr : tbits, two_partials ? nullptr : ubits, obits,
                                      h, w, c->bits_stride, n, nbits1, nbits2);
      if (!opened && !u8_mask && n <= 4)
          opened = launch_or_open5_small(s, mbits, partials ? ebits : nullptr, (!partials || two_partials) ? nullptr : tbits,
                                         (!partials || two_partials) ? nullptr : ubits, obits, h, w, c->bits_stride, n, nbits1, nbits2);
      if (!opened) {
          if (partials) launch_or4_bits(s, mbits, ebits, two_partials ? ebits : tbits, two_partials ? ebits : ubits, h, w, c->bits_stride, n, nbits1, nbits2);
          if (u8_mask) launch_open5_bits(s, mbits, ebits, mask, h, w, ps, c->bits_stride, n);
          else launch_open5_to_bits(s, mbits, ebits, obits, h, w, c->bits_stride, n);
      } }
    (void)t0;
    HIP_TRY(hipGetLastError());
    return LT_OK;
}

int make_search_geom(lt_ctx* c, const lt_search_params* p, bool band, SearchGeom& g) {
    if (!p) return fail(LT_ERR_INVALID, "null search params");
    const int h = c->calib.warp_h, w = c->calib.warp_w;
    std::memset(&g, 0, sizeof g);
    g.h = h;
    g.w = w;
    if (p->ignore_bottom < 0 || p->ignore_bottom > h) return fail(LT_ERR_INVALID, "ignore_bottom out of range");
    if (!(p->partial >= 0.0 && p->partial <= 1.0)) return fail(LT_ERR_INVALID, "partial must be in [0,1]");
// ... 115 lines not shown
    if (it == sp.out.end()) return;
    sp.idle[it->second].push_back(st);
    sp.out.erase(it);
}

hipError_t create_compute_stream(hipStream_t* st, int reserved) { return stream_get(st, SK_COMPUTE, reserved); }

}

extern "C" {

const char* lt_last_error(void) { return g_err.c_str(); }
int lt_abi_version(void) { return LT_ABI_VERSION; }

int lt_device_count(int* count) {
    if (!count) return fail(LT_ERR_INVALID, "null count");
    HIP_TRY(hipGetDeviceCount(count));
    return LT_OK;
}

const char* lt_stage_name(int stage) { return stage >= 0 && stage < LT_NUM_STAGES ? kStageNames[stage] : ""; }

int lt_create(const lt_calib* calib, int device, lt_ctx** out) {
    if (!calib || !out) return fail(LT_ERR_INVALID, "null argument");
    if (calib->img_w < 2 || calib->img_h < 2 || calib->warp_w < 2 || calib->warp_h < 2 || calib->img_w > 16384 ||
        calib->img_h > 16384 || calib->warp_w > 4096 || calib->warp_h > 16384)
        return fail(LT_ERR_INVALID, "camera size must be in [2, 16384], bird's-eye width in [2, 4096], height in [2, 16384]");
    int ndev = 0;
    HIP_TRY(hipGetDeviceCount(&ndev));
    if (ndev <= 0) return fail(LT_ERR_HIP, "no HIP device visible: the lane-tracker kernels need a GPU (gfx950)");
    if (device < 0 || device >= ndev) return fail(LT_ERR_INVALID, "device %d out of range (%d visible)", device, ndev);
    TraceScope ts_all("lt_create");
    lt_ctx* c = new lt_ctx();
    c->calib = *calib;
    c->device = device;
    auto bail = [&](int rc) {
        lt_destroy(c);
        return rc;
    };
    if (const char* e = LT_EXP_ENV("LT_WALK_MIN_FRAMES")) c->walk_min_pixels = atoll(e) * calib->warp_w * calib->warp_h;
    if (hipSetDevice(device) != hipSuccess) return bail(fail(LT_ERR_HIP, "hipSetDevice(%d) failed", device));
    if (hipGetDeviceProperties(&c->prop, device) != hipSuccess) return bail(fail(LT_ERR_HIP, "hipGetDeviceProperties failed"));
    if (create_compute_stream(&c->stream) != hipSuccess) return bail(fail(LT_ERR_HIP, "hipStreamCreate failed"));
    c->streams.assign(1, c->stream);
    c->nstreams = 1;
    if (hipEventCreate(&c->ev0) != hipSuccess || hipEventCreate(&c->ev1) != hipSuccess) return bail(fail(LT_ERR_HIP, "hipEventCreate failed"));
    if (stream_get(&c->copy, SK_PLAIN, 0) != hipSuccess) return bail(fail(LT_ERR_HIP, "copy stream creation failed"));

    const double t_tables = trace_on() ? trace_now() : 0.0;
    RemapTable warp, und;
    build_warp_table(*calib, warp);
    int r0 = 0, r1 = 0;
    warp_source_rows(*calib, warp, r0, r1);
    build_undistort_table(*calib, r0, r1, und);
    c->fe = FrontEndGeom{calib->img_h, calib->img_w, calib->warp_h, calib->warp_w, r0, r1 - r0};
    {
        int lo = calib->img_h, hi = 0;
        for (size_t o = 0; o < (size_t)und.rows * und.cols; ++o) {
            const int sx = und.xy[o * 2], sy = und.xy[o * 2 + 1];
            if (sy < -1 || sy >= calib->img_h || sx < -1 || sx >= calib->img_w) continue;
            lo = std::min(lo, std::max(sy, 0));
            hi = std::max(hi, std::min(sy + 2, calib->img_h));
        }
        c->cam_r0 = hi > lo ? lo : 0;
        c->cam_r1 = hi > lo ? hi : 0;
    }
    uint16_t gamma_tab[256], cbrt_tab[3072];
    int32_t coef[9];
    build_lab_tables(gamma_tab, cbrt_tab, coef);
    auto make_se = [](int k, EllipseSE& se) {
        int dx[64];
        ellipse_halfwidths(k, dx);
        se.k = k;
        for (int i = 0; i < 64; ++i) se.dx[i] = (int8_t)(i < k ? dx[i] : 0);
    };
    make_se(5, c->se5);
    make_se(29, c->se29);
    make_se(55, c->se55);
    if (!tophat_tables_match(c->se29, c->se55))
        return bail(fail(LT_ERR_STATE, "compiled-in ellipse run tables disagree with getStructuringElement's formula"));
    {
        const char* e = LT_EXP_ENV("LT_TOPHAT_BRUTE");
        c->brute_tophat = e && e[0] == '1';
    }

    if (trace_on()) trace_line("lt_create:host_tables", t_tables);
    TraceScope ts_up("lt_create:table_upload");
    int rc;
    if ((rc = dev_alloc(&c->d_wxy, warp.xy.size()))) return bail(rc);
    if ((rc = dev_alloc(&c->d_wfrac, warp.frac.size()))) return bail(rc);
    if ((rc = dev_alloc(&c->d_uxy, und.xy.size()))) return bail(rc);
    if ((rc = dev_alloc(&c->d_ufrac, und.frac.size()))) return bail(rc);
    if ((rc = dev_alloc(&c->d_gamma, 256))) return bail(rc);
    if ((rc = dev_alloc(&c->d_cbrt, 3072))) return bail(rc);
    if ((rc = dev_alloc(&c->d_coef, 9))) return bail(rc);
    hipError_t e = hipSuccess;
    auto up = [&](void* dst, const void* src, size_t bytes) {
        if (e == hipSuccess && bytes) e = hipMemcpy(dst, src, bytes, hipMemcpyHostToDevice);
    };
    up(c->d_wxy, warp.xy.data(), warp.xy.size() * 2);
    up(c->d_wfrac, warp.frac.data(), warp.frac.size() * 2);
    up(c->d_uxy, und.xy.data(), und.xy.size() * 2);
    up(c->d_ufrac, und.frac.data(), und.frac.size() * 2);
    up(c->d_gamma, gamma_tab, sizeof gamma_tab);
    up(c->d_cbrt, cbrt_tab, sizeof cbrt_tab);
    up(c->d_coef, coef, sizeof coef);
    if (e != hipSuccess) return bail(fail(LT_ERR_HIP, "table upload failed: %s", hipGetErrorString(e)));

    preload_kernels(device, c->stream);
    c->frame_bytes = (size_t)calib->img_h * calib->img_w * 3;
    c->yuv_bytes = c->frame_bytes / 2;
    c->yuv_stride = (c->yuv_bytes + 15) & ~(size_t)15;
    c->und_bytes = (size_t)c->fe.nrows * calib->img_w * 3;
    c->und_px = (size_t)c->fe.nrows * calib->img_w;
    c->plane_bytes = (size_t)calib->warp_h * calib->warp_w;
    c->bev_bytes = c->plane_bytes * 3;
    *out = c;
    return LT_OK;
}

void lt_destroy(lt_ctx* c) {
    if (!c) return;
    (void)hipSetDevice(c->device);
    static const bool trace = std::getenv("LT_TRACE_DESTROY") != nullptr;
    auto note = [&](const char* what) { if (trace) { std::fprintf(stderr, "lt_destroy: %s\n", what); std::fflush(stderr); } };
    note("streams of the slots");
    for (auto st : c->streams) if (st) (void)hipStreamSynchronize(st);
    {
        const char* names[5] = {"copy", "search", "present", "urgent", "dl"};
        hipStream_t sts[5] = {c->copy, c->search, c->present, c->urgent, c->dl};
        for (int i = 0; i < 5; ++i) if (sts[i]) { note(names[i]); (void)hipStreamSynchronize(sts[i]); }
    }
    note("events: timing pool, order ring, staging");
    for (auto e : c->ev_pool) (void)hipEventDestroy(e);
    for (auto e : c->order_events) (void)hipEventDestroy(e);
    if (c->spans_busy.done) (void)hipEventDestroy(c->spans_busy.done);
    if (c->text_busy.done) (void)hipEventDestroy(c->text_busy.done);
    if (c->annot_busy.done) (void)hipEventDestroy(c->annot_busy.done);
    note("streams back to the pool: dl");
    stream_put(c->dl);
    note("events: download timing");
    for (auto& d : c->dl_inflight) { (void)hipEventDestroy(d.a); (void)hipEventDestroy(d.b); }
    for (auto e : c->dl_event_pool) (void)hipEventDestroy(e);
    note("streams back to the pool: present, urgent");
    stream_put(c->present);
    stream_put(c->urgent);
    if (c->rest_done) (void)hipEventDestroy(c->rest_done);
    note("hipHostFree(spans, lines, xpos)");
    if (c->h_spans) (void)hipHostFree(c->h_spans);
    if (c->h_lines) (void)hipHostFree(c->h_lines);
    if (c->h_xpos) (void)hipHostFree(c->h_xpos);
    note("events: slot-range rings, chain tickets");
    for (auto& w : c->readers.e) if (w.ev) (void)hipEventDestroy(w.ev);
    for (auto& w : c->writers.e) if (w.ev) (void)hipEventDestroy(w.ev);
    for (auto& w : c->rests.e) if (w.ev) (void)hipEventDestroy(w.ev);
    for (auto& w : c->yuv_rows.e) if (w.ev) (void)hipEventDestroy(w.ev);
    for (auto& t : c->chains) (void)hipEventDestroy(t.done);
    for (auto e : c->chain_event_pool) (void)hipEventDestroy(e);
    note("hipHostFree(small, rec, rec_stage, cancel)");
    if (c->h_small) (void)hipHostFree(c->h_small);
    if (c->h_lists) (void)hipHostFree(c->h_lists);
    if (c->h_rec) (void)hipHostFree(c->h_rec);
    if (c->h_rec_stage) (void)hipHostFree(c->h_rec_stage);
    if (c->h_cancel) (void)hipHostFree(c->h_cancel);
    if (c->h_items) (void)hipHostFree(c->h_items);
    if (c->items_ev) (void)hipEventDestroy(c->items_ev);
// ... 674 lines not shown
}

int lt_download_plane(lt_ctx* c, int plane, int first, int n, uint8_t* out) {
    int rc = check_slots(c, first, n);
    if (rc) return rc;
    static const int map[6] = {P_R, P_B, P_THR, P_THB, P_MERGED, P_MASK};
    if (plane < 0 || plane > 5) return fail(LT_ERR_INVALID, "unknown plane %d", plane);
    if (plane == LT_PLANE_MASK) {
        if ((rc = set_device(c))) return rc;
        if ((rc = ensure_u8_masks(c, first, n))) return rc;
    }
    if (plane == LT_PLANE_MERGED) {
        if ((rc = set_device(c))) return rc;
        if ((rc = sync_all(c))) return rc;
        if ((rc = ensure_plane(c, P_MERGED))) return rc;
        launch_bits_to_u8(c->stream, c->d_bits_merged + (size_t)first * c->bits_stride,
                          c->d_plane[P_MERGED] + (size_t)first * c->plane_bytes, c->calib.warp_h, c->calib.warp_w,
                          c->plane_bytes, c->bits_stride, n);
    }
    if (plane == LT_PLANE_TOPHAT_R || plane == LT_PLANE_TOPHAT_B) {
        if (!out) return fail(LT_ERR_INVALID, "null output buffer");
        if ((rc = set_device(c))) return rc;
        if ((rc = sync_all(c))) return rc;
        const int w = c->calib.warp_w, h = c->calib.warp_h, q = plane == LT_PLANE_TOPHAT_R ? 0 : 1;
        for (int i = first; i < first + n; ++i) {
            uint8_t* dst = out + (size_t)(i - first) * c->plane_bytes;
            if (i < (int)c->th_padded.size() && c->th_padded[(size_t)i])
                HIP_TRY(hipMemcpy2DAsync(dst, (size_t)w, c->d_th_pad[q] + (size_t)i * c->th_pad_bytes, (size_t)c->th_pitch, (size_t)w,
                                         (size_t)h, hipMemcpyDeviceToHost, c->stream));
            else
                HIP_TRY(hipMemcpyAsync(dst, c->d_plane[map[plane]] + (size_t)i * c->plane_bytes, c->plane_bytes,
                                       hipMemcpyDeviceToHost, c->stream));
        }
        HIP_TRY(hipStreamSynchronize(c->stream));
        return LT_OK;
    }
    return download(c, c->d_plane[map[plane]] + (size_t)first * c->plane_bytes, out, (size_t)n * c->plane_bytes);
}

int lt_download_undistorted(lt_ctx* c, int first, int n, uint8_t* out) {
    int rc = check_slots(c, first, n);
    if (rc) return rc;
    if (!out) return fail(LT_ERR_INVALID, "null output buffer");
    if (n == 0 || c->und_bytes == 0) return LT_OK;
    if ((rc = set_device(c))) return rc;
    uint8_t* tmp = nullptr;
    if ((rc = sync_all(c))) return rc;
    if ((rc = dev_alloc(&tmp, (size_t)n * c->und_bytes))) return rc;
    launch_undistorted_to_rgb(c->stream, c->d_und, c->und_px, first, c->fe.nrows, c->fe.img_w, tmp, n);
    rc = download(c, tmp, out, (size_t)n * c->und_bytes);
    dev_free(tmp);
    return rc;
}

int lt_calib_source_rows(const lt_calib* calib, int* row0, int* row1) {
    if (!calib || !row0 || !row1) return fail(LT_ERR_INVALID, "null argument");
    RemapTable warp;
    build_warp_table(*calib, warp);
    warp_source_rows(*calib, warp, *row0, *row1);
    return LT_OK;
}

int lt_calib_warp_table(const lt_calib* calib, int16_t* xy, uint16_t* frac) {
    if (!calib || !xy || !frac) return fail(LT_ERR_INVALID, "null argument");
    RemapTable t;
    build_warp_table(*calib, t);
    const size_t n = (size_t)t.rows * t.cols;
    std::memcpy(xy, t.xy.data(), n * 2 * sizeof(int16_t));
    std::memcpy(frac, t.frac.data(), n * sizeof(uint16_t));
    return LT_OK;
}

int lt_calib_undistort_table(const lt_calib* calib, int row0, int row1, int16_t* xy, uint16_t* frac) {
    if (!calib || !xy || !frac) return fail(LT_ERR_INVALID, "null argument");
    if (row0 < 0 || row1 < row0 || row1 > calib->img_h) return fail(LT_ERR_INVALID, "rows [%d, %d) outside the image", row0, row1);
    RemapTable t;
    build_undistort_table(*calib, row0, row1, t);
    const size_t n = (size_t)t.rows * t.cols;
    std::memcpy(xy, t.xy.data(), n * 2 * sizeof(int16_t));
    std::memcpy(frac, t.frac.data(), n * sizeof(uint16_t));
    return LT_OK;
}

int lt_calib_lab_tables(uint16_t* gamma256, uint16_t* cbrt3072, int32_t* coeffs9) {
    if (!gamma256 || !cbrt3072 || !coeffs9) return fail(LT_ERR_INVALID, "null argument");
    build_lab_tables(gamma256, cbrt3072, coeffs9);
    return LT_OK;
}

int lt_calib_ellipse(int k, int32_t* halfwidths, int* taps) {
    if (k < 1 || k > 63 || !(k & 1) || !halfwidths || !taps) return fail(LT_ERR_INVALID, "k must be odd, 1..63");
    int dx[64];
    *taps = ellipse_halfwidths(k, dx);
    for (int i = 0; i < k; ++i) halfwidths[i] = dx[i];
    return LT_OK;
}

static lt_lane_record* rec_mirror_device(lt_ctx* c) {
    if (!c->h_rec && hipHostMalloc(reinterpret_cast<void**>(&c->h_rec), 256, hipHostMallocDefault) != hipSuccess) {
        (void)hipGetLastError();
        c->h_rec = nullptr;
    } else if (c->h_rec && !c->rec_ticket_counter) {
        std::memset(c->h_rec, 0, 256);
        c->rec_ticket_counter = 1;
    }
    void* dev = nullptr;
    if (!c->h_rec || hipHostGetDevicePointer(&dev, c->h_rec, 0) != hipSuccess) {
        (void)hipGetLastError();
        return nullptr;
    }
    return static_cast<lt_lane_record*>(dev);
}
static void mirror_record(lt_ctx* c, hipStream_t st, int slot) {
    c->rec_mirror_slot = -1;
    c->rec_ticket = 0;
    static_assert(sizeof(lt_lane_record) == 64, "k_mirror_record copies 16 words and stores the ticket behind them");
    unsigned ticket = ++c->rec_ticket_counter;
    if (!ticket) ticket = ++c->rec_ticket_counter;
    if (rec_mirror_device(c) && launch_mirror_record(st, c->h_rec, slot_rec(c, slot), ticket)) {
        c->rec_mirror_slot = slot;
        c->rec_mirror_stream = st;
        c->rec_ticket = ticket;
    }
}

int lt_download_records(lt_ctx* c, int first, int n, lt_lane_record* out) {
    int rc = check_slots(c, first, n);
    if (rc) return rc;
    if (n == 1 && out && c->rec_mirror_slot == first && c->h_rec) {
        if ((rc = set_device(c))) return rc;
        static const bool poll = [] { const char* e = LT_EXP_ENV("LT_RECORD_POLL"); return !(e && e[0] == '0'); }();
        bool seen = false;
        if (poll && c->rec_ticket) {
            const volatile unsigned* word = reinterpret_cast<const volatile unsigned*>(c->h_rec + 1);
            const auto t0 = std::chrono::steady_clock::now();
            for (unsigned spins = 0; !(seen = *word == c->rec_ticket); ++spins) {
                __builtin_ia32_pause();
                if ((spins & 1023u) == 1023u && std::chrono::steady_clock::now() - t0 > std::chrono::milliseconds(2)) break;
            }
            std::atomic_thread_fence(std::memory_order_acquire);
        }
        if (!seen) HIP_TRY(hipStreamSynchronize(c->rec_mirror_stream));
        std::memcpy(out, c->h_rec, sizeof(lt_lane_record));
        return LT_OK;
    }
    return download(c, slot_rec(c, first), out, (size_t)n * sizeof(lt_lane_record));
}

static int expand_pixels(const lt_ctx* c, const lt_lane_record& r, const uint32_t* region, size_t region_words, int side, int32_t* ys,
                         int32_t* xs, int cap, int* count) {
    if (r._pad == 1) {
        const int nlev = (int)region[0], wh = (int)region[1], H1 = (int)region[2];
        const long long words = sws2_block_words(nlev, wh);
        if (nlev < 1 || wh < 1 || words > (long long)region_words) return fail(LT_ERR_STATE, "corrupt lane-pixel block");
        const int32_t* roi = reinterpret_cast<const int32_t*>(region + 4);
        const uint32_t* masks = region + sws2_mask_offset(nlev);
        int n = 0;
        for (int level = 0; level < nlev; ++level) {
            const int sl = side * nlev + level, a = roi[sl * 2], b = roi[sl * 2 + 1];
            if (b <= a) continue;
            for (int ry = 0; ry < wh; ++ry) {
                const size_t mi = ((size_t)sl * wh + ry) * 2;
                unsigned long long m = (unsigned long long)masks[mi] | ((unsigned long long)masks[mi + 1] << 32);
                const int y = H1 - (1 + level) * wh + ry;
                while (m) {
                    const int j = __builtin_ctzll(m);
// ... 118 lines not shown
}

int lt_download_centroids(lt_ctx* c, int slot, int side, int32_t* out, int cap, int* count) {
    int rc = check_slots(c, slot, 1);
    if (rc) return rc;
    if (side < 0 || side > 1 || !count || cap < 0 || (cap > 0 && !out)) return fail(LT_ERR_INVALID, "bad side/count/cap/out");
    if (!c->d_cent) return fail(LT_ERR_STATE, "no sliding-window search has run yet");
    std::vector<int32_t> tmp((size_t)c->maxlev + 2);
    if ((rc = download(c, slot_cent(c, slot) + (size_t)side * (c->maxlev + 2), tmp.data(), tmp.size() * 4))) return rc;
    int n = tmp[0];
    if (n < 0) n = 0;
    if (n > c->maxlev + 1) n = c->maxlev + 1;
    *count = n;
    for (int i = 0; i < n && i < cap; ++i) out[i] = tmp[1 + i];
    return LT_OK;
}

int lt_copy_records_to_device(lt_ctx* c, int first, int n, void* dst) {
    int rc = check_slots(c, first, n);
    if (rc) return rc;
    if (!dst) return fail(LT_ERR_INVALID, "null destination");
    if ((rc = set_device(c))) return rc;
    if ((rc = sync_all(c))) return rc;
    HIP_TRY(hipMemcpyAsync(dst, slot_rec(c, first), (size_t)n * sizeof(lt_lane_record), hipMemcpyDeviceToDevice, c->stream));
    HIP_TRY(hipStreamSynchronize(c->stream));
    return LT_OK;
}

int lt_enqueue_records_to_device(lt_ctx* c, int first, int n, void* dst) {
    int rc = check_slots(c, first, n);
    if (rc) return rc;
    if (!dst) return fail(LT_ERR_INVALID, "null destination");
    if ((rc = set_device(c))) return rc;
    rc = for_each_slice(c, first, n, [&](hipStream_t st, int f0, int m) {
        HIP_TRY(hipMemcpyAsync(static_cast<lt_lane_record*>(dst) + (f0 - first), slot_rec(c, f0), (size_t)m * sizeof(lt_lane_record),
                               hipMemcpyDeviceToDevice, st));
        return (int)LT_OK;
    });
    return rc;
}

int lt_set_frame_base(lt_ctx* c, int first, int n, int first_frame) {
    int rc = check_slots(c, first, n);
    if (rc) return rc;
    c->rec_mirror_slot = -1;
    if ((rc = set_device(c))) return rc;
    std::vector<lt_lane_record> tmp((size_t)n);
    if (n == 0) return LT_OK;
    if ((rc = download(c, slot_rec(c, first), tmp.data(), tmp.size() * sizeof(lt_lane_record)))) return rc;
    for (int i = 0; i < n; ++i) tmp[i].frame = first_frame + i;
    HIP_TRY(hipMemcpyAsync(slot_rec(c, first), tmp.data(), tmp.size() * sizeof(lt_lane_record), hipMemcpyHostToDevice, c->stream));
    HIP_TRY(hipStreamSynchronize(c->stream));
    return LT_OK;
}

static int mask_run_impl(lt_ctx* c, int first, int n, const lt_filter_params* p, bool reuse_front) {
    int rc = check_slots(c, first, n);
    if (rc) return rc;
    if ((rc = validate_filter(p))) return rc;
    if ((rc = set_device(c))) return rc;
    if (n == 0) return LT_OK;
    const size_t ps = c->plane_bytes;
    rc = for_each_slice(c, first, n, [&](hipStream_t st, int f0, int m) {
        bool have_front = reuse_front && !c->stage_timing && f0 + m <= (int)c->front_ok.size();
        for (int i = f0; have_front && i < f0 + m; ++i) have_front = c->front_ok[(size_t)i] != 0;
        if (!have_front) {
            { StageScope t(c, ST_UNDISTORT, st);
              auto is_attached = [&](int i) { return i < (int)c->attached.size() && c->attached[(size_t)i] != 0; };
              for (int a = f0, b; a < f0 + m; a = b) {
                  const bool att = is_attached(a);
                  for (b = a + 1; b < f0 + m && is_attached(b) == att; ++b) {}
                  const FrameSource src = att ? FrameSource::surfaces(c->d_surf)
                                          : c->in_layout != LT_INPUT_RGB ? FrameSource::slots(slot_yuv(c, a), c->yuv_stride)
                                                                         : FrameSource::slots(slot_frame(c, a), c->frame_bytes);
                  launch_undistort_rows(st, src, c->in_layout, yuv_coef_of(c), c->d_uxy, c->d_ufrac, c->fe, c->d_und, c->und_px, a, b - a);
              } }
            { int mrc = n == 1 ? note_range_frame(c, c->readers, st, f0, f0 + m) : note_range(c->readers, st, f0, f0 + m); if (mrc) return mrc; }
            { StageScope t(c, ST_WARP_SPLIT, st);
              launch_warp_split(st, c->d_und, c->und_px, f0, c->d_wxy, c->d_wfrac, c->fe, c->d_gamma,
                                c->d_cbrt, c->d_coef, c->d_plane[P_R] + (size_t)f0 * ps, c->d_plane[P_B] + (size_t)f0 * ps,
                                ps, m); }
            for (int i = f0; i < f0 + m && i < (int)c->front_ok.size(); ++i) c->front_ok[(size_t)i] = 1;
        }
        int frc = run_filter_chain(c, st, f0, m, p, c->calib.warp_h, c->calib.warp_w, n);
        return frc ? frc : note_written_frame(c, st, f0, f0 + m, n);
    });
    if (rc) return rc;
    c->have_mask = true;
    mark_masks(c, first, n, 1, 0);
    return LT_OK;
}

int lt_mask_run(lt_ctx* c, int first, int n, const lt_filter_params* p) { return mask_run_impl(c, first, n, p, false); }
int lt_mask_rerun(lt_ctx* c, int first, int n, const lt_filter_params* p) { return mask_run_impl(c, first, n, p, true); }

int lt_filter_run(lt_ctx* c, int first, int n, const lt_filter_params* p) {
    int rc = check_slots(c, first, n);
    if (rc) return rc;
    if ((rc = validate_filter(p))) return rc;
    if ((rc = set_device(c))) return rc;
    if (!c->d_bev) return fail(LT_ERR_STATE, "lt_upload_bev has not been called");
    if (n == 0) return LT_OK;
    const size_t ps = c->plane_bytes;
    front_stale(c, first, n);
    rc = for_each_slice(c, first, n, [&](hipStream_t st, int f0, int m) {
        { StageScope t(c, ST_SPLIT_BEV, st);
          launch_split_bev(st, c->d_bev + (size_t)f0 * c->bev_bytes, c->bev_bytes, (int)ps, c->d_gamma, c->d_cbrt,
                           c->d_coef, c->d_plane[P_R] + (size_t)f0 * ps, c->d_plane[P_B] + (size_t)f0 * ps, ps, m); }
        int frc = run_filter_chain(c, st, f0, m, p, c->calib.warp_h, c->calib.warp_w, n);
        return frc ? frc : note_written(c, st, f0, f0 + m);
    });
    if (rc) return rc;
    c->have_mask = true;
    mark_masks(c, first, n, 1, 0);
    return LT_OK;
}

static void launch_sws_slots(lt_ctx* c, hipStream_t st, const SearchGeom& g, const MaskBits& mb, int f0, int m) {
    launch_sws_fit(st, slot_mask(c, f0), c->plane_bytes, mb, g, slot_band_sums(c, f0, g.nbands), slot_pix(c, f0), slot_cent(c, f0),
                   slot_rec(c, f0), m);
}
static void launch_band_slots(lt_ctx* c, hipStream_t st, const SearchGeom& g, const BandPrev& bp, const MaskBits& mb, int f0, int m) {
    launch_band_fit(st, slot_mask(c, f0), c->plane_bytes, mb, g, slot_prev(c, f0), bp, slot_pix(c, f0), slot_rec(c, f0), m);
}

int lt_sws_fit_run(lt_ctx* c, int first, int n, const lt_search_params* p) {
    int rc = check_slots(c, first, n);
    if (rc) return rc;
    c->rec_mirror_slot = -1;
    if ((rc = set_device(c))) return rc;
    if (!c->have_mask) return fail(LT_ERR_STATE, "no mask in the slots: run lt_mask_run or lt_upload_masks first");
    SearchGeom g;
    if ((rc = prepare_search(c, p, false, g))) return rc;
    if (n == 0) return LT_OK;
    const bool use_bits = slot_reads_bits(c, g, 0, first, n);
    if (!use_bits && (rc = ensure_u8_masks(c, first, n))) return rc;
    rc = for_each_slice(c, first, n, [&](hipStream_t st, int f0, int m) {
        StageScope t(c, ST_SWS_FIT, st);
        launch_sws_slots(c, st, g, slot_bits(c, f0, use_bits), f0, m);
        if (n == 1) mirror_record(c, st, f0);
        return note_written_frame(c, st, f0, f0 + m, n);
    });
    if (rc) return rc;
    HIP_TRY(hipGetLastError());
    return LT_OK;
}

int lt_band_fit_run(lt_ctx* c, int first, int n, const lt_search_params* p, const double* prev) {
    int rc = check_slots(c, first, n);
    if (rc) return rc;
    c->rec_mirror_slot = -1;
    if (!prev) return fail(LT_ERR_INVALID, "band search needs the previous coefficients (last_left_coeffs/last_right_coeffs)");
    if ((rc = set_device(c))) return rc;
    if (!c->have_mask) return fail(LT_ERR_STATE, "no mask in the slots: run lt_mask_run or lt_upload_masks first");
    SearchGeom g;
    if ((rc = prepare_search(c, p, true, g))) return rc;
    if (n == 0) return LT_OK;
    BandPrev bp;
    std::memset(&bp, 0, sizeof bp);
    bool one_seed = true;
    for (int i = 1; i < n && one_seed; ++i) one_seed = std::memcmp(prev, prev + (size_t)i * 6, 6 * sizeof(double)) == 0;
    if (one_seed) {
        std::memcpy(bp.c, prev, sizeof bp.c);
        bp.by_value = 1;
    } else {
        if ((rc = sync_all(c))) return rc;
        HIP_TRY(hipMemcpyAsync(slot_prev(c, first), prev, (size_t)n * 6 * sizeof(double), hipMemcpyHostToDevice, c->stream));
// ... 456 lines not shown
```

lane_tracker_amd/csrc/lt_ctx.h:

```cpp
#pragma once
#include <hip/hip_runtime.h>

#include <algorithm>
#include <functional>
#include <memory>
#include <vector>

#include "lt_internal.h"

namespace lt {

int fail(int code, const char* fmt, ...) __attribute__((format(printf, 2, 3)));

#define HIP_TRY(expr)                                                                               \
    do {                                                                                            \
        hipError_t e_ = (expr);                                                                     \
        if (e_ != hipSuccess) return lt::fail(LT_ERR_HIP, "%s failed: %s", #expr, hipGetErrorString(e_)); \
    } while (0)

enum Stage {
    ST_UNDISTORT = 0, ST_WARP_SPLIT, ST_ERODE_R, ST_TOPHAT_R, ST_ERODE_B, ST_TOPHAT_B, ST_THRESHOLD, ST_MERGE,
    ST_OPEN, ST_SWS_FIT, ST_BAND_FIT, ST_SPLIT_BEV
};

enum Plane { P_R = 0, P_B, P_THR, P_THB, P_MERGED, P_MASK, P_T0, P_T1, P_T2, P_T3, P_COUNT };

}

using lt::P_COUNT;

struct lt_ctx {
    lt_calib calib{};
    int device = 0;
    hipStream_t stream = nullptr;
    std::vector<hipStream_t> streams;
    hipStream_t copy = nullptr;
    int direct_upload = -1;
    bool direct_upload_wanted = true;
    unsigned long long lane_spec_reader_seq = 0;
    unsigned long long direct_uploads = 0;
    int nstreams = 1;
    hipDeviceProp_t prop{};
    lt::FrontEndGeom fe{};
    int cam_r0 = 0, cam_r1 = 0;
    lt::EllipseSE se5{}, se29{}, se55{};
    int16_t *d_uxy = nullptr, *d_wxy = nullptr;
    uint16_t *d_ufrac = nullptr, *d_wfrac = nullptr, *d_gamma = nullptr, *d_cbrt = nullptr;
    int32_t* d_coef = nullptr;
    int capacity = 0;
    size_t frame_bytes = 0, und_bytes = 0, plane_bytes = 0, bev_bytes = 0;
    uint8_t *d_frames = nullptr, *d_bev = nullptr;
    int in_layout = 0;
    int32_t yuv_coef[5] = {0, 0, 0, 0, 0};
    bool input_locked = false;
    uint8_t* d_yuv = nullptr;
    size_t yuv_bytes = 0, yuv_stride = 0;
    lt::SurfEntry* d_surf = nullptr;
    std::vector<lt::SurfEntry> surf;
    std::vector<uint8_t> attached;
    uint32_t* d_und = nullptr;
    size_t und_px = 0;
    uint8_t* d_plane[P_COUNT] = {};
    uint8_t* d_side_scratch = nullptr;
    unsigned long long *d_bits_merged = nullptr, *d_bits_eroded = nullptr;
    unsigned long long* d_bits_open = nullptr;
    unsigned long long* d_bits_tmp = nullptr;
    unsigned long long* d_bits_tmp2 = nullptr;
    uint8_t* d_th_pad[2] = {nullptr, nullptr};
    size_t th_pad_bytes = 0;
    int th_pitch = 0;
    std::vector<uint8_t> th_padded;
    uint8_t* d_b_pad = nullptr;
    unsigned long long *d_bits_n1 = nullptr, *d_bits_n2 = nullptr;
    int last_threshold_path = -1;
    int last_adaptive_path = -1;
    long long walk_min_pixels = 80LL * 1100 * 1080;
    std::vector<uint8_t> mask_bits_ok, mask_u8_ok;
    std::vector<uint8_t> frame_full, annot_full;
    std::vector<uint8_t> front_ok;
    size_t bits_stride = 0;
    lt_lane_record* d_rec = nullptr;
    double* d_prev = nullptr;
    uint32_t* d_pix = nullptr;
    int32_t* d_cent = nullptr;
    uint32_t* d_band_sums = nullptr;
    lt_search_item* d_items = nullptr;
    lt_search_item* h_items = nullptr;
    int items_cap = 0;
    hipEvent_t items_ev = nullptr;
    int maxpix = 0, maxlev = 0, maxbands = 0;
    bool have_mask = false;
    bool brute_tophat = false;
    int16_t* d_oxy = nullptr;
    uint16_t* d_ofrac = nullptr;
    bool have_overlay = false;
    int16_t* d_spans = nullptr;
    uint8_t* d_annot = nullptr;
    uint8_t* d_strip = nullptr;
    size_t strip_bytes = 0;
    int16_t* h_spans = nullptr;
    int h_spans_cap = 0;
    struct StagingBusy { int lo = 0, hi = 0; hipEvent_t done = nullptr; };
    StagingBusy spans_busy, text_busy;
    hipStream_t dl = nullptr;
    hipStream_t present = nullptr;
    double* d_ploty = nullptr;
    std::vector<double> h_ploty;
    hipStream_t lane_spec_stream = nullptr;
    unsigned lane_spec_ticket = 0;
    hipStream_t urgent = nullptr;
    bool urgent_on = false;
    StagingBusy annot_busy;
    struct DlTimed { hipEvent_t a, b; double bytes; int method; };
    std::vector<DlTimed> dl_inflight;
    std::vector<hipEvent_t> dl_event_pool;
    double dl_rate[2] = {0.0, 0.0};
    int dl_samples[2] = {0, 0};
    int dl_method = 0;
    int dl_since_probe = 0;
    int dl_forced = -1;
    hipEvent_t rest_done = nullptr;
    bool rest_pending = false;
    uint8_t *d_atlas = nullptr, *d_advance = nullptr, *d_lines = nullptr;
    int16_t* d_xpos = nullptr;
    std::vector<uint8_t> h_advance;
    uint8_t* h_lines = nullptr;
    int16_t* h_xpos = nullptr;
    int font_first = 0, font_glyphs = 0, font_gw = 0, font_gh = 0;
    size_t text_per_slot = 0;
    int text_slots = 0;
    std::vector<hipEvent_t> order_events;
    size_t order_next = 0;
    struct RangeEvents {
        struct Entry { int lo, hi; hipEvent_t ev; };
        std::vector<Entry> e = std::vector<Entry>(32, Entry{0, 0, nullptr});
        unsigned head = 0, count = 0;
        bool overflow = false;
        bool lazy = false;
        unsigned long long lazy_seq = 0, lazy_seen = 0;
        void reset() { head = count = 0; overflow = false; lazy = false; lazy_seen = lazy_seq; }
    };
    RangeEvents readers, writers;
    RangeEvents yuv_rows;
    RangeEvents rests;
    hipStream_t search = nullptr;
    int search_cus = 0;
    struct ChainTicket { int first, n; hipEvent_t done; int own; };
    std::vector<ChainTicket> chains;
    std::vector<hipEvent_t> chain_event_pool;
    int* h_cancel = nullptr;
    int* d_cancel = nullptr;
    uint8_t* h_small = nullptr;
    uint8_t* h_lists = nullptr;
    size_t h_lists_bytes = 0;
    int ov_r0 = 0, ov_r1 = 0;
    lt_lane_record* h_rec = nullptr;
    int rec_mirror_slot = -1;
    hipStream_t rec_mirror_stream = nullptr;
    unsigned rec_ticket = 0, rec_ticket_counter = 0;
    lt_lane_record* h_rec_stage = nullptr;
    int h_rec_stage_cap = 0;
    hipEvent_t ev0 = nullptr, ev1 = nullptr;
    bool stage_timing = false;
    std::vector<hipEvent_t> ev_pool;
    struct Pending { int stage; hipEvent_t a, b; };
    std::vector<Pending> pending;
    size_t ev_used = 0;
    float stage_ms[LT_NUM_STAGES] = {};
    int32_t stage_launches[LT_NUM_STAGES] = {};
};

namespace lt {

inline uint8_t* slot_frame(const lt_ctx* c, int s) { return c->d_frames + (size_t)s * c->frame_bytes; }
inline uint8_t* slot_yuv(const lt_ctx* c, int s) { return c->d_yuv + (size_t)s * c->yuv_stride; }
// ... 174 lines not shown
```

lane_tracker_amd/csrc/lt_internal.h:

```cpp
#pragma once
#include <hip/hip_runtime.h>
#include <stdint.h>

#include <vector>

#include <cstdlib>

#include "../../include/lane_tracker_amd.h"

#ifdef LT_EXPERIMENTS
#define LT_EXP_ENV(name) std::getenv(name)
#else
#define LT_EXP_ENV(name) (static_cast<const char*>(nullptr))
#endif

namespace lt {

struct RemapTable {
    std::vector<int16_t> xy;
    std::vector<uint16_t> frac;
    int rows = 0, cols = 0;
};
void build_warp_table(const lt_calib& c, RemapTable& t);
void warp_source_rows(const lt_calib& c, const RemapTable& warp, int& r0, int& r1);
void build_undistort_table(const lt_calib& c, int r0, int r1, RemapTable& t);
void build_lab_tables(uint16_t gamma_tab[256], uint16_t cbrt_tab[3072], int32_t coeffs[9]);
int  ellipse_halfwidths(int k, int* dx);

struct EllipseSE {
    int k;
    int8_t dx[64];
};

struct FrontEndGeom {
    int img_h, img_w, warp_h, warp_w, r0, nrows;
};
#if defined(__HIPCC__)
__host__ __device__
#endif
inline size_t und_slot_base(size_t und_px, int slot) { return (size_t)(slot >> 1) * 2 * und_px + (size_t)(slot & 1); }
void launch_warp_split(hipStream_t s, const uint32_t* und, size_t und_px, int first_slot, const int16_t* wxy,
                       const uint16_t* wfrac, FrontEndGeom g, const uint16_t* gamma_tab, const uint16_t* cbrt_tab,
                       const int32_t* coeffs, uint8_t* planeR, uint8_t* planeB, size_t plane_stride, int n);
struct YuvCoef {
    int32_t cy, cvr, cvg, cug, cub;
};
void launch_yuv_rows_to_rgb(hipStream_t s, int layout, const uint8_t* yuv, size_t yuv_stride, YuvCoef k, uint8_t* rgb,
                            size_t rgb_stride, int h, int w, int r0, int r1, int n);
struct SurfEntry {
    uint64_t plane[3];
    int32_t pitch, cpitch;
};
static_assert(sizeof(SurfEntry) == 32, "SurfEntry: 32 bytes, two scalar loads");
struct SurfChunk {
    static constexpr int N = 32;
    SurfEntry e[N];
};
struct FrameSource {
    const SurfEntry* tab;
    const uint8_t* frames;
    size_t stride;
    static FrameSource slots(const uint8_t* frames, size_t stride) { return FrameSource{nullptr, frames, stride}; }
    static FrameSource surfaces(const SurfEntry* tab) { return FrameSource{tab, nullptr, 0}; }
};
void launch_undistort_rows(hipStream_t s, FrameSource src, int layout, YuvCoef k, const int16_t* uxy, const uint16_t* ufrac,
                           FrontEndGeom g, uint32_t* und, size_t und_px, int first_slot, int n);
void launch_write_surf_entries(hipStream_t s, SurfEntry* tab, int first, const SurfEntry* entries, int n);
void launch_surf_rows_to_rgb(hipStream_t s, int layout, const SurfEntry* entries, YuvCoef k, uint8_t* rgb, size_t rgb_stride, int w,
                             int r0, int r1, int n);
void launch_split_bev(hipStream_t s, const uint8_t* bev, size_t bev_stride, int npix, const uint16_t* gamma_tab,
                      const uint16_t* cbrt_tab, const int32_t* coeffs, uint8_t* planeR, uint8_t* planeB,
                      size_t plane_stride, int n);
void launch_undistorted_to_rgb(hipStream_t s, const uint32_t* und, size_t und_px, int first_slot, int nrows, int w, uint8_t* out,
                               int n);

void preload_k_frontend(hipStream_t s);
void preload_k_filter(hipStream_t s);
void preload_k_tophat(hipStream_t s);
void preload_k_threshold(hipStream_t s);
void preload_k_threshold_walk(hipStream_t s);
void preload_k_adaptive_walk(hipStream_t s);
void preload_k_search(hipStream_t s);
void preload_k_overlay(hipStream_t s);

bool launch_overlay_lane_strip(hipStream_t s, const uint8_t* frames, size_t frame_stride, uint8_t* strips, size_t strip_stride,
                               const int16_t* oxy, const uint16_t* ofrac, const int16_t* spans, size_t span_stride_rows, int img_w,
                               int row0, int row1, int bh, int bw, float alpha, int n);
void launch_overlay_lane(hipStream_t s, const uint8_t* frames, uint8_t* out, size_t frame_stride, const int16_t* oxy,
                         const uint16_t* ofrac, const int16_t* spans, size_t span_stride_rows, int img_h, int img_w,
                         int bh, int bw, float alpha, int n, const int* rows4 = nullptr);
constexpr int LT_SPAN_ARG_ROWS = 1104;
void launch_store_word(hipStream_t s, unsigned* dev_word, unsigned value);
bool launch_lane_spans_from_regions(hipStream_t s, const double* ploty, const double* ploty2, int n_rows, int bh, int bw, int16_t* spans, int n);
bool launch_lane_spans_from_fit(hipStream_t s, const lt_lane_record* rec, const double* prev_sum, int count, const double* ploty,
                                const double* ploty2, int n_rows, int bh, int bw, int16_t* spans);
bool launch_overlay_lane_one(hipStream_t s, const uint8_t* frame, uint8_t* out, const int16_t* oxy, const uint16_t* ofrac,
                             const int16_t* spans_host, int img_h, int img_w, int bh, int bw, float alpha, const int* rows4);
void launch_overlay_text(hipStream_t s, uint8_t* out, size_t frame_stride, int img_h, int img_w, const uint8_t* atlas,
                         const uint8_t* advance, int first_char, int n_glyphs, int gw, int gh, const uint8_t* lines,
                         const int16_t* xpos, int nl, int len, int slot_chars, int y0, int step, int n);
void launch_copy_from_pinned(hipStream_t s, void* dst, const void* src_pinned, size_t bytes);
bool launch_copy_to_pinned(hipStream_t s, void* dst_pinned, const void* src, size_t bytes);
bool launch_copy_rows_to_pinned(hipStream_t s, void* dst_pinned, const void* src, size_t pitch, size_t off, size_t bytes, int n);
bool launch_copy_words_to_pinned(hipStream_t s, void* dst_pinned, const void* src, size_t bytes);
bool launch_mirror_record(hipStream_t s, void* dst_pinned, const void* src_record, unsigned ticket);
void launch_warp_rgb(hipStream_t s, const uint32_t* und, size_t und_px, int first_slot, const int16_t* wxy, const uint16_t* wfrac,
                     FrontEndGeom g, uint8_t* bev, size_t bev_stride, int n);

void launch_morph_ellipse(hipStream_t s, const uint8_t* src, uint8_t* dst, const uint8_t* minuend, int h, int w,
                          const EllipseSE& se, bool dilate, size_t plane_stride, int n);
bool launch_morph_runs(hipStream_t s, const uint8_t* src, uint8_t* dst, const uint8_t* minuend, int h, int w, int k,
                       bool dilate, size_t plane_stride, int n, int dpitch = 0, size_t dst_stride = 0, uint8_t* copy_dst = nullptr);
bool launch_morph_one_pair(hipStream_t s, const uint8_t* src55, uint8_t* dst55, const uint8_t* min55, const uint8_t* src29, uint8_t* dst29,
                           const uint8_t* min29, int h, int w, bool dilate, size_t plane_stride, int n, int dpitch, size_t dst_stride);
bool tophat_tables_match(const EllipseSE& se29, const EllipseSE& se55);
void launch_bilateral(hipStream_t s, const uint8_t* src, uint8_t* dst, int h, int w, int ksize, int C, int mode,
                      int tv, int fv, size_t plane_stride, int n);
void launch_adaptive_mean(hipStream_t s, const uint8_t* src, uint8_t* dst, int h, int w, int bs, int C,
                          size_t plane_stride, int n);
bool adaptive_walk_supported(int bs_r, int bs_b, int h, int w, size_t plane_stride);
bool launch_adaptive_walk(hipStream_t s, const uint8_t* R, int bs_r, int C_r, unsigned long long* out_r, const uint8_t* B, int bs_b,
                          int C_b, unsigned long long* out_b, int h, int w, size_t plane_stride, size_t bits_stride, int n);
void launch_merge(hipStream_t s, const uint8_t* tr, const uint8_t* tb, const uint8_t* labb, const uint8_t* noise_bil,
                  int noise_thresh, int use_noise, uint8_t* merged, size_t npix, size_t plane_stride, int n);

int launch_bilateral_bits(hipStream_t s, const uint8_t* thr, int k_r, int C_r, const uint8_t* thb, int k_b, int C_b,
                          const uint8_t* labb, int k_n, int C_n, int noise_thresh, int use_noise,
                          unsigned long long* bits, int h, int w, size_t plane_stride, size_t bits_stride, int n,
                          unsigned long long* bits_v = nullptr);
void launch_pack_merge(hipStream_t s, const uint8_t* tr, const uint8_t* tb, const uint8_t* labb, const uint8_t* nb,
                       int noise_thresh, int use_noise, unsigned long long* bits, int h, int w, size_t plane_stride,
                       size_t bits_stride, int n);
void launch_open5_bits(hipStream_t s, const unsigned long long* merged, unsigned long long* eroded, uint8_t* mask, int h,
                       int w, size_t plane_stride, size_t bits_stride, int n);
bool bilateral_walk_supported(int k_r, int C_r, int k_b, int C_b, int h, int w, int pitch);
int launch_bilateral_walk(hipStream_t s, const uint8_t* thr, int k_r, int C_r, const uint8_t* thb, int k_b, int C_b,
                          unsigned long long* merged, unsigned long long* s1, unsigned long long* s2, unsigned long long* s3,
                          int h, int w, int pitch, size_t plane_stride, size_t bits_stride, int n, bool merge);
void launch_or4_bits(hipStream_t s, unsigned long long* merged, const unsigned long long* s1, const unsigned long long* s2,
                     const unsigned long long* s3, int h, int w, size_t bits_stride, int n, const unsigned long long* n0 = nullptr,
                     const unsigned long long* n1 = nullptr);
bool noise_walk_supported(int k_n, int C_n, int h, int w, int pitch);
int launch_noise_walk(hipStream_t s, const uint8_t* braw, int k_n, int C_n, int noise_thresh, unsigned long long* noise_h,
                      unsigned long long* noise_v, int h, int w, int pitch, size_t plane_stride, size_t bits_stride, int n);
bool launch_merge_open5(hipStream_t s, unsigned long long* p0, const unsigned long long* p1, const unsigned long long* p2,
                        const unsigned long long* p3, unsigned long long* opened, int h, int w, size_t bits_stride, int n,
                        const unsigned long long* n0 = nullptr, const unsigned long long* n1 = nullptr);
bool launch_or_open5_small(hipStream_t s, unsigned long long* p0, const unsigned long long* p1, const unsigned long long* p2,
                        const unsigned long long* p3, unsigned long long* opened, int h, int w, size_t bits_stride, int n,
                        const unsigned long long* n0 = nullptr, const unsigned long long* n1 = nullptr);
void launch_open5_to_bits(hipStream_t s, const unsigned long long* merged, unsigned long long* eroded,
                          unsigned long long* opened, int h, int w, size_t bits_stride, int n);
void launch_bits_to_u8(hipStream_t s, const unsigned long long* bits, uint8_t* out, int h, int w, size_t plane_stride,
                       size_t bits_stride, int n);


struct SearchGeom {
    int h, w;
    int ww, wh, hw;
    int img_height;
    int img_center, y_start, nlevels, limit;
    int nbands;
    int ignore_sides, search_range, def_left, def_right;
    int band_top, band_bottom;
    double mu, bandwidth;
    int maxpix, maxlev;
};
__host__ __device__ inline int sws2_mask_offset(int nlev) { return (4 + 4 * nlev + 1) & ~1; }
__host__ __device__ inline long long sws2_block_words(int nlev, int wh) { return sws2_mask_offset(nlev) + 4LL * nlev * wh; }
__host__ __device__ inline int band2_mask_offset(int nrows) { return (4 + 2 * nrows + 1) & ~1; }
__host__ __device__ inline long long band2_block_words(int nrows) { return band2_mask_offset(nrows) + 4LL * nrows; }
__host__ __device__ inline size_t band2_mom_offset(int nrows) { return ((size_t)2 * nrows * 16 + 16 + 15) & ~(size_t)15; }
struct MaskBits {
    const unsigned long long* bits;
    size_t bits_stride;
    int wpr;
};
bool sws_fit_takes_bits(const SearchGeom& g, size_t mask_stride);
bool band_fit_takes_bits(const SearchGeom& g, size_t mask_stride);
void launch_sws_fit(hipStream_t s, const uint8_t* masks, size_t mask_stride, MaskBits mb, SearchGeom g, uint32_t* band_sums,
                    uint32_t* pix, int32_t* cent, lt_lane_record* rec, int n);
struct BandPrev {
    double c[6];
    int by_value;
};
void launch_band_fit(hipStream_t s, const uint8_t* masks, size_t mask_stride, MaskBits mb, SearchGeom g, const double* prev,
                     const BandPrev& bp, uint32_t* pix, lt_lane_record* rec, int n);

bool band_chain_supported(const SearchGeom& g, size_t mask_stride);
bool launch_band_fit_one(hipStream_t s, MaskBits mb, SearchGeom g, const BandPrev& bp, uint32_t* pix, lt_lane_record* rec,
                         size_t mask_stride, const int* zero, lt_lane_record* mirror, unsigned mirror_ticket);
void launch_band_chain(hipStream_t s, const uint8_t* masks, size_t mask_stride, MaskBits mb, SearchGeom g, const lt_lane_record* seed_rec,
                       const BandPrev& seed, uint32_t* pix, lt_lane_record* rec, int n, const int* cancel_epoch, int my_epoch);

bool search_list_supported(const SearchGeom* gs, const SearchGeom* gb, size_t mask_stride);
// ... 17 lines not shown
```

lane_tracker_amd/csrc/lt_tables.cpp:

```cpp
#include <cfloat>
#include <climits>
#include <cmath>
#include <cstring>

#include "lt_internal.h"

namespace lt {
namespace {

constexpr int kInterBits = 5;
constexpr int kInterTab = 1 << kInterBits;

inline int cv_round(double v) {
    if (!(v > (double)INT_MIN)) return INT_MIN;
    if (!(v < (double)INT_MAX)) return INT_MAX;
    return (int)std::nearbyint(v);
}
inline int16_t clamp_s16(int v) { return (int16_t)(v < SHRT_MIN ? SHRT_MIN : (v > SHRT_MAX ? SHRT_MAX : v)); }

struct Mat3 {
    double m[9];
    double operator()(int r, int c) const { return m[r * 3 + c]; }
};

bool invert3(const Mat3& a, Mat3& out) {
    const double c00 = a(1, 1) * a(2, 2) - a(1, 2) * a(2, 1);
    const double c01 = a(1, 0) * a(2, 2) - a(1, 2) * a(2, 0);
    const double c02 = a(1, 0) * a(2, 1) - a(1, 1) * a(2, 0);
    double det = a(0, 0) * c00 - a(0, 1) * c01 + a(0, 2) * c02;
    if (det == 0.0) return false;
    const double id = 1.0 / det;
    out.m[0] = c00 * id;
    out.m[1] = (a(0, 2) * a(2, 1) - a(0, 1) * a(2, 2)) * id;
    out.m[2] = (a(0, 1) * a(1, 2) - a(0, 2) * a(1, 1)) * id;
    out.m[3] = (a(1, 2) * a(2, 0) - a(1, 0) * a(2, 2)) * id;
    out.m[4] = (a(0, 0) * a(2, 2) - a(0, 2) * a(2, 0)) * id;
    out.m[5] = (a(0, 2) * a(1, 0) - a(0, 0) * a(1, 2)) * id;
    out.m[6] = c02 * id;
    out.m[7] = (a(0, 1) * a(2, 0) - a(0, 0) * a(2, 1)) * id;
    out.m[8] = (a(0, 0) * a(1, 1) - a(0, 1) * a(1, 0)) * id;
    return true;
}

inline void store_fixed(RemapTable& t, size_t o, int X, int Y, bool saturate) {
    int sx = X >> kInterBits, sy = Y >> kInterBits;
    t.xy[o * 2] = saturate ? clamp_s16(sx) : (int16_t)sx;
    t.xy[o * 2 + 1] = saturate ? clamp_s16(sy) : (int16_t)sy;
    t.frac[o] = (uint16_t)((Y & (kInterTab - 1)) * kInterTab + (X & (kInterTab - 1)));
}

}

void build_warp_table(const lt_calib& c, RemapTable& t) {
    Mat3 M, m;
    std::memcpy(M.m, c.M, sizeof M.m);
    if (!invert3(M, m)) std::memset(m.m, 0, sizeof m.m);
    t.rows = c.warp_h;
    t.cols = c.warp_w;
    t.xy.assign((size_t)t.rows * t.cols * 2, 0);
    t.frac.assign((size_t)t.rows * t.cols, 0);
    constexpr int kBlockW = 64;
    for (int y = 0; y < t.rows; ++y)
        for (int x0 = 0; x0 < t.cols; x0 += kBlockW) {
            const double X0 = m.m[0] * x0 + m.m[1] * y + m.m[2];
            const double Y0 = m.m[3] * x0 + m.m[4] * y + m.m[5];
            const double W0 = m.m[6] * x0 + m.m[7] * y + m.m[8];
            const int bw = t.cols - x0 < kBlockW ? t.cols - x0 : kBlockW;
            for (int x1 = 0; x1 < bw; ++x1) {
                double w = W0 + m.m[6] * x1;
                w = w != 0.0 ? kInterTab / w : 0.0;
                double fx = (X0 + m.m[0] * x1) * w, fy = (Y0 + m.m[3] * x1) * w;
                fx = std::fmax((double)INT_MIN, std::fmin((double)INT_MAX, fx));
                fy = std::fmax((double)INT_MIN, std::fmin((double)INT_MAX, fy));
                store_fixed(t, (size_t)y * t.cols + x0 + x1, cv_round(fx), cv_round(fy), true);
            }
        }
}

void warp_source_rows(const lt_calib& c, const RemapTable& warp, int& r0, int& r1) {
    int lo = INT_MAX, hi = INT_MIN;
    const size_t n = (size_t)warp.rows * warp.cols;
    for (size_t o = 0; o < n; ++o) {
        const int sx = warp.xy[o * 2], sy = warp.xy[o * 2 + 1];
        if (sx + 1 < 0 || sx >= c.img_w) continue;
        for (int yy = sy; yy <= sy + 1; ++yy)
            if (yy >= 0 && yy < c.img_h) {
                lo = yy < lo ? yy : lo;
                hi = yy > hi ? yy : hi;
            }
    }
    if (lo > hi) {
        r0 = r1 = 0;
        return;
    }
    r0 = lo;
    r1 = hi + 1;
}

void build_undistort_table(const lt_calib& c, int r0, int r1, RemapTable& t) {
    const int w = c.img_w;
    int stripe = 4096 / (w > 1 ? w : 1);
    stripe = stripe < 1 ? 1 : (stripe > c.img_h ? c.img_h : stripe);
    t.rows = r1 - r0;
    t.cols = w;
    t.xy.assign((size_t)t.rows * w * 2 + 2, 0);
    t.frac.assign((size_t)t.rows * w + 1, 0);
    const double fx = c.cam_matrix[0], fy = c.cam_matrix[4], u0 = c.cam_matrix[2], v0 = c.cam_matrix[5];
    const double k1 = c.dist_coeffs[0], k2 = c.dist_coeffs[1], p1 = c.dist_coeffs[2], p2 = c.dist_coeffs[3],
                 k3 = c.dist_coeffs[4];
    int cached_origin = -1;
    Mat3 ir{};
    for (int row = r0; row < r1; ++row) {
        const int origin = row - row % stripe, i = row - origin;
        if (origin != cached_origin) {
            Mat3 Ar;
            std::memcpy(Ar.m, c.cam_matrix, sizeof Ar.m);
            Ar.m[5] = c.cam_matrix[5] - origin;
            invert3(Ar, ir);
            cached_origin = origin;
        }
        double xn = i * ir.m[1] + ir.m[2], yn = i * ir.m[4] + ir.m[5], wn = i * ir.m[7] + ir.m[8];
        for (int j = 0; j < w; ++j) {
            const double iw = 1. / wn, x = xn * iw, y = yn * iw;
            const double x2 = x * x, y2 = y * y, r2 = x2 + y2, xy2 = 2 * x * y;
            const double kr = 1 + ((k3 * r2 + k2) * r2 + k1) * r2;
            const double xd = x * kr + p1 * xy2 + p2 * (r2 + 2 * x2);
            const double yd = y * kr + p1 * (r2 + 2 * y2) + p2 * xy2;
            const double u = fx * xd + u0, v = fy * yd + v0;
            store_fixed(t, (size_t)(row - r0) * w + j, cv_round(u * kInterTab), cv_round(v * kInterTab), false);
            xn += ir.m[0];
            yn += ir.m[3];
            wn += ir.m[6];
        }
    }
}

void build_lab_tables(uint16_t gamma_tab[256], uint16_t cbrt_tab[3072], int32_t coeffs[9]) {
    auto to_u16 = [](float v) {
        int r = cv_round((double)v);
        return (uint16_t)(r < 0 ? 0 : (r > 65535 ? 65535 : r));
    };
    for (int i = 0; i < 256; ++i) {
        const float x = i * (1.f / 255.f);
        const float lin = x <= 0.04045f ? x * (1.f / 12.92f) : (float)std::pow((double)(x + 0.055) * (1. / 1.055), 2.4);
        gamma_tab[i] = to_u16(255.f * (1 << 3) * lin);
    }
    for (int i = 0; i < 3072; ++i) {
        const float x = i * (1.f / (255.f * (1 << 3)));
        const float f = x < 0.008856f ? x * 7.787f + 0.13793103448275862f : (float)std::cbrt((double)x);
        cbrt_tab[i] = to_u16((1 << 15) * f);
    }
    const float rgb2xyz[9] = {0.412453f, 0.357580f, 0.180423f, 0.212671f, 0.715160f,
                              0.072169f, 0.019334f, 0.119193f, 0.950227f};
    const float white[3] = {0.950456f, 1.f, 1.088754f};
    for (int r = 0; r < 3; ++r) {
        const float scale = r == 1 ? (float)(1 << 12) : (1 << 12) / white[r];
        for (int col = 0; col < 3; ++col) coeffs[r * 3 + col] = cv_round((double)(rgb2xyz[r * 3 + col] * scale));
    }
}

int ellipse_halfwidths(int k, int* dx) {
    const int r = k / 2;
    const double inv_r2 = r ? 1. / ((double)r * r) : 0.;
    int taps = 0;
    for (int i = 0; i < k; ++i) {
        const int dy = i - r;
        int d = cv_round(r * std::sqrt((r * r - dy * dy) * inv_r2));
        dx[i] = d;
        const int j1 = r - d > 0 ? r - d : 0, j2 = r + d + 1 < k ? r + d + 1 : k;
        taps += j2 - j1;
    }
    return taps;
}

}
```

Before: 98350 frames/s.

## Cull morphology tasks to live bird's-eye rows derived from the warp table

Uses the warp table to find which bird's-eye pixels can ever map to valid source pixels, then builds per-strip row ranges (widened by the structuring-element margin) and runs the erode/top-hat tasks only over those ranges. Task lists are cached on device and sorted longest first. Rows outside the live range are filled directly, with zero for the top-hat or the source value for the erode, instead of running full morphology. This removes work on regions that are always dead after the perspective warp. The cost is a table lookup per task and extra fill stores, and the culling is on by default only when the frames were warped in the same call.

```diff
diff --git a/include/lane_tracker_amd.h b/include/lane_tracker_amd.h
--- a/include/lane_tracker_amd.h
+++ b/include/lane_tracker_amd.h
@@ -234,6 +234,8 @@
 int  lt_calib_undistort_table(const lt_calib* calib, int row0, int row1, int16_t* xy, uint16_t* frac);
 int  lt_calib_lab_tables(uint16_t* gamma256, uint16_t* cbrt3072, int32_t* coeffs9);
 int  lt_calib_ellipse(int k, int32_t* halfwidths , int* taps);
+int  lt_live_tasks(const lt_calib* calib, int k, int stage, int window, int cull, int band_rows, int32_t* tasks, int cap, int* n_tasks,
+                   int* n_pair, int32_t* strip_rows, double* dead_fraction);
 
 typedef struct lt_gather lt_gather;
 int  lt_gather_init(lt_ctx* ctx, int rank, int world, const char* id_path, int timeout_s, lt_gather** out);
diff --git a/lane_tracker_amd/_native.py b/lane_tracker_amd/_native.py
--- a/lane_tracker_amd/_native.py
+++ b/lane_tracker_amd/_native.py
@@ -173,6 +173,8 @@
     "lt_calib_undistort_table": (C.c_int, [C.POINTER(Calib), C.c_int, C.c_int, _P, _P]),
     "lt_calib_lab_tables": (C.c_int, [_P, _P, _P]),
     "lt_calib_ellipse": (C.c_int, [C.c_int, _P, C.POINTER(C.c_int)]),
+    "lt_live_tasks": (C.c_int, [C.POINTER(Calib), C.c_int, C.c_int, C.c_int, C.c_int, C.c_int, _P, C.c_int, C.POINTER(C.c_int),
+                                C.POINTER(C.c_int), _P, C.POINTER(C.c_double)]),
     "lt_gather_init": (C.c_int, [_P, C.c_int, C.c_int, C.c_char_p, C.c_int, C.POINTER(_P)]),
     "lt_gather_world": (C.c_int, [_P, C.POINTER(C.c_int), C.POINTER(C.c_int)]),
     "lt_gather_reserve": (C.c_int, [_P, C.c_int]),
@@ -535,6 +537,17 @@
                 cbrt=cbrt, lab_coeffs=coef, ellipse=ell)
 
 
+def live_tasks(cal, k, stage, window=0, cull=True, band_rows=0):
+    lib = load()
+    nstrips = (cal.warp_w + 127) // 128
+    cap = nstrips * (cal.warp_h + 1)
+    tasks, rows = np.zeros((cap, 4), np.int32), np.zeros((nstrips, 2), np.int32)
+    n, npair, dead = C.c_int(0), C.c_int(0), C.c_double(0.0)
+    _check(lib.lt_live_tasks(C.byref(cal), int(k), int(stage), int(window), int(bool(cull)), int(band_rows), tasks.ctypes.data, cap,
+                             C.byref(n), C.byref(npair), rows.ctypes.data, C.byref(dead)))
+    return dict(tasks=tasks[:n.value].copy(), n_pair=npair.value, strip_rows=rows, dead_fraction=dead.value)
+
+
 def pack_polygons(polygons):
     ln = np.array([len(p[0]) for p in polygons], np.int32)
     rn = np.array([len(p[2]) for p in polygons], np.int32)
diff --git a/lane_tracker_amd/csrc/k_tophat.hip b/lane_tracker_amd/csrc/k_tophat.hip
--- a/lane_tracker_amd/csrc/k_tophat.hip
+++ b/lane_tracker_amd/csrc/k_tophat.hip
@@ -122,6 +122,8 @@
     int n_normal;
     int xcd;
     uint8_t* copy_dst;
+    const LiveTask* tasks = nullptr;
+    int ntab = 0, ntab_pair = 0;
 };
 
 struct LaneCols {
@@ -476,7 +478,8 @@
 
 template <class SE, bool DIL, bool WIDE, bool TH, bool PAIR, bool COPYM = false>
 __device__ __forceinline__ void morph_task(const uint8_t* __restrict__ src, uint8_t* __restrict__ dst, const uint8_t* __restrict__ minuend,
-                                           const RunsGeom& g, uint2* chain, uint8_t* s_out_w, int lane, int strip, int band, int frame) {
+                                           const RunsGeom& g, uint2* chain, uint8_t* s_out_w, int lane, int strip, int yb0, int yb1, int fill,
+                                           int frame) {
     static_assert(WIDE || !PAIR, "pair strips exist for the WIDE kernels only");
     static_assert(!COPYM || (WIDE && TH), "the minuend copy rides on the dword store of the WIDE top-hat");
     constexpr int K = SE::K, R = SE::R, NH = SE::NH;
@@ -487,7 +490,6 @@
     const bool has_b = PAIR && frame + 1 < g.nframes;
     const bool lane_b = PAIR && (lane & 16);
     const int x0 = strip * 128;
-    const int yb0 = band * g.band_rows, yb1 = min(yb0 + g.band_rows, g.h);
     const int xa = x0 + lane, xb = xa + 64;
     const bool va = xa < g.w, vb = xb < g.w;
     const int oa = min(xa, g.w - 1), ob = min(xb, g.w - 1);
@@ -653,6 +655,41 @@
         out_issue(q);
         out_finish(q, mcur, y_tail);
     }
+    if constexpr (WIDE) {
+        if (fill) {
+            constexpr int LPR = PAIR ? 16 : 32, RPI = 64 / LPR;
+            const int fcol = x0 + 4 * (lane & (LPR - 1));
+            const int nfr = has_b ? 2 : 1;
+#pragma unroll 1
+            for (int part = 0; part < 2; ++part) {
+                if (!(fill & (1 << part))) continue;
+                const int ra = part ? yb1 : 0, rb = part ? g.h : yb0;
+                if (fcol >= g.w) continue;
+                constexpr int FU = 8;
+#pragma unroll 1
+                for (int fr = 0; fr < nfr; ++fr)
+#pragma unroll 1
+                    for (int r = ra + lane / LPR; r < rb; r += FU * RPI) {
+                        uint32_t v[FU], mv[FU];
+#pragma unroll
+                        for (int u = 0; u < FU; ++u) {
+                            const size_t so = (size_t)fr * g.plane_stride + (size_t)min(r + u * RPI, g.h - 1) * g.w + fcol;
+                            v[u] = TH ? 0u : *reinterpret_cast<const uint32_t*>(s + so);
+                            mv[u] = COPYM ? *reinterpret_cast<const uint32_t*>(m + so) : 0u;
+                        }
+                        asm volatile("" : "+v"(v[0]), "+v"(v[1]), "+v"(v[2]), "+v"(v[3]), "+v"(v[4]), "+v"(v[5]), "+v"(v[6]), "+v"(v[7]),
+                                          "+v"(mv[0]), "+v"(mv[1]), "+v"(mv[2]), "+v"(mv[3]), "+v"(mv[4]), "+v"(mv[5]), "+v"(mv[6]), "+v"(mv[7]));
+#pragma unroll
+                        for (int u = 0; u < FU; ++u) {
+                            if (r + u * RPI >= rb) break;
+                            const size_t dof = (size_t)fr * g.dst_stride + (size_t)(r + u * RPI) * g.dpitch + fcol;
+                            *reinterpret_cast<uint32_t*>(d + dof) = v[u];
+                            if (COPYM) *reinterpret_cast<uint32_t*>(g.copy_dst + (size_t)frame * g.dst_stride + dof) = mv[u];
+                        }
+                    }
+            }
+        }
+    }
 }
 
 #ifndef LT_MORPH_WPB
@@ -678,14 +715,28 @@
     if (task >= g.ntasks) return;
     if (!LT_MORPH_BIAS) __builtin_amdgcn_s_setreg(1 | (6 << 6) | (1 << 11), 3);
     const int n_pair = g.ntasks - g.n_normal;
-    if (!WIDE || task >= n_pair) {
-        const int t = task - n_pair;
-        const int strip = t % g.nstrips_normal;
-        const int band = (t / g.nstrips_normal) % g.nbands;
-        const int frame = t / (g.nstrips_normal * g.nbands);
-        morph_task<SE, DIL, WIDE, TH, false, COPYM>(src, dst, minuend, g, s_chain[wv], s_out[wv], lane, strip, band, frame);
+    const bool pair = WIDE && task < n_pair;
+    int strip, yb0, yb1, frame, fill = 0;
+    if (WIDE && g.tasks) {
+        const int t = pair ? task : task - n_pair, per = pair ? g.ntab_pair : g.ntab;
+        const LiveTask e = g.tasks[(pair ? 0 : g.ntab_pair) + t % per];
+        frame = pair ? 2 * (t / per) : t / per;
+        strip = e.strip;
+        yb0 = e.y0;
+        yb1 = e.y0 + e.rows;
+        fill = e.flags;
+    } else {
+        const int t = pair ? task : task - n_pair;
+        const int band = pair ? t % g.nbands : (t / g.nstrips_normal) % g.nbands;
+        strip = pair ? g.nstrips_normal : t % g.nstrips_normal;
+        frame = pair ? 2 * (t / g.nbands) : t / (g.nstrips_normal * g.nbands);
+        yb0 = band * g.band_rows;
+        yb1 = min(yb0 + g.band_rows, g.h);
+    }
+    if (!pair) {
+        morph_task<SE, DIL, WIDE, TH, false, COPYM>(src, dst, minuend, g, s_chain[wv], s_out[wv], lane, strip, yb0, yb1, fill, frame);
     } else if constexpr (WIDE) {
-        morph_task<SE, DIL, WIDE, TH, true, COPYM>(src, dst, minuend, g, s_chain[wv], s_out[wv], lane, g.nstrips_normal, task % g.nbands, 2 * (task / g.nbands));
+        morph_task<SE, DIL, WIDE, TH, true, COPYM>(src, dst, minuend, g, s_chain[wv], s_out[wv], lane, strip, yb0, yb1, fill, frame);
     }
 }
 
@@ -860,7 +911,7 @@
 
 template <class SE>
 bool launch_runs(hipStream_t s, const uint8_t* src, uint8_t* dst, const uint8_t* minuend, int h, int w, bool dilate,
-                 size_t plane_stride, int n, int dpitch, size_t dst_stride, uint8_t* copy_dst) {
+                 size_t plane_stride, int n, int dpitch, size_t dst_stride, uint8_t* copy_dst, LiveTaskCache* live) {
     RunsGeom g;
     g.copy_dst = copy_dst;
     g.h = h;
@@ -926,6 +977,15 @@
     g.nstrips_normal = pair_strip ? g.nstrips - 1 : g.nstrips;
     g.n_normal = n * g.nstrips_normal * g.nbands;
     g.ntasks = g.n_normal + (pair_strip ? (n + 1) / 2 * g.nbands : 0);
+    if (live && wide && !one_row && ((uintptr_t)src & 3) == 0) {
+        if (const LiveTable* t = live->get(dilate ? 2 * SE::R : SE::R, std::min(2 * SE::R, h), g.band_rows, pair_strip)) {
+            g.tasks = t->d_tasks;
+            g.ntab = t->n_normal;
+            g.ntab_pair = t->n_pair;
+            g.n_normal = n * g.ntab;
+            g.ntasks = g.n_normal + (n + 1) / 2 * g.ntab_pair;
+        }
+    }
     static const bool want_xcd = [] { const char* e = LT_EXP_ENV("LT_MORPH_XCD"); return e && e[0] == '1'; }();
     g.xcd = want_xcd ? 1 : 0;
     dim3 grid((g.ntasks + 3) / 4);
@@ -967,11 +1027,11 @@
 }
 
 bool launch_morph_runs(hipStream_t s, const uint8_t* src, uint8_t* dst, const uint8_t* minuend, int h, int w, int k,
-                       bool dilate, size_t plane_stride, int n, int dpitch, size_t dst_stride, uint8_t* copy_dst) {
+                       bool dilate, size_t plane_stride, int n, int dpitch, size_t dst_stride, uint8_t* copy_dst, LiveTaskCache* live) {
     if (n <= 0 || h <= 0 || w <= 0) return true;
     if (k == 55)
-        return launch_runs<SE55>(s, src, dst, minuend, h, w, dilate, plane_stride, n, dpitch, dst_stride, copy_dst);
-    return launch_runs<SE29>(s, src, dst, minuend, h, w, dilate, plane_stride, n, dpitch, dst_stride, copy_dst);
+        return launch_runs<SE55>(s, src, dst, minuend, h, w, dilate, plane_stride, n, dpitch, dst_stride, copy_dst, live);
+    return launch_runs<SE29>(s, src, dst, minuend, h, w, dilate, plane_stride, n, dpitch, dst_stride, copy_dst, live);
 }
 
 bool launch_morph_one_pair(hipStream_t s, const uint8_t* src55, uint8_t* dst55, const uint8_t* min55, const uint8_t* src29, uint8_t* dst29,
diff --git a/lane_tracker_amd/csrc/lt_api.cpp b/lane_tracker_amd/csrc/lt_api.cpp
--- a/lane_tracker_amd/csrc/lt_api.cpp
+++ b/lane_tracker_amd/csrc/lt_api.cpp
@@ -361,8 +361,10 @@
 constexpr int SIDE_LANES = 10;
 
 int run_filter_chain(lt_ctx* c, hipStream_t s, int first, int n, const lt_filter_params* p, int h, int w, int call_frames,
-                     bool u8_mask = false) {
+                     bool u8_mask = false, bool warped_here = false) {
     const size_t ps = c->plane_bytes, off = (size_t)first * ps;
+    LiveTaskCache* const tasks = c->live_tasks.rows.h != h || c->live_tasks.rows.w != w ? nullptr
+                                 : warped_here && c->live_tasks_on ? &c->live_tasks : &c->full_tasks;
     uint8_t* R = c->d_plane[P_R] + off;
     uint8_t* B = c->d_plane[P_B] + off;
     uint8_t* thR = c->d_plane[P_THR] + off;
@@ -391,8 +393,8 @@
     uint8_t* thRd = walk ? c->d_th_pad[0] + (size_t)first * c->th_pad_bytes : thR;
     uint8_t* thBd = walk ? c->d_th_pad[1] + (size_t)first * c->th_pad_bytes : thB;
     auto tophat_b = [&](hipStream_t st) -> int {
-        if (bpad && launch_morph_runs(st, t0, thBd, B, h, w, 55, true, ps, n, dpitch, c->th_pad_bytes, bpad)) return LT_OK;
-        launch_morph_runs(st, t0, thBd, B, h, w, 55, true, ps, n, dpitch, c->th_pad_bytes);
+        if (bpad && launch_morph_runs(st, t0, thBd, B, h, w, 55, true, ps, n, dpitch, c->th_pad_bytes, bpad, tasks)) return LT_OK;
+        launch_morph_runs(st, t0, thBd, B, h, w, 55, true, ps, n, dpitch, c->th_pad_bytes, nullptr, tasks);
         if (bpad)
             for (int i = 0; i < n; ++i)
                 HIP_TRY(hipMemcpy2DAsync(bpad + (size_t)i * c->th_pad_bytes, (size_t)c->th_pitch, B + (size_t)i * ps, (size_t)w, (size_t)w,
@@ -431,9 +433,9 @@
             }
             both_split = !p->mask_noise;
         } else {
-            { StageScope t(c, ST_ERODE_R, s);  launch_morph_runs(s, R, t0, nullptr, h, w, 29, false, ps, n); }
-            { StageScope t(c, ST_TOPHAT_R, s); launch_morph_runs(s, t0, thRd, R, h, w, 29, true, ps, n, dpitch, c->th_pad_bytes); }
-            { StageScope t(c, ST_ERODE_B, s);  launch_morph_runs(s, B, t0, nullptr, h, w, 55, false, ps, n); }
+            { StageScope t(c, ST_ERODE_R, s);  launch_morph_runs(s, R, t0, nullptr, h, w, 29, false, ps, n, 0, 0, nullptr, tasks); }
+            { StageScope t(c, ST_TOPHAT_R, s); launch_morph_runs(s, t0, thRd, R, h, w, 29, true, ps, n, dpitch, c->th_pad_bytes, nullptr, tasks); }
+            { StageScope t(c, ST_ERODE_B, s);  launch_morph_runs(s, B, t0, nullptr, h, w, 55, false, ps, n, 0, 0, nullptr, tasks); }
             { StageScope t(c, ST_TOPHAT_B, s); const int rc = tophat_b(s); if (rc) return rc; }
         }
     }
@@ -715,6 +717,12 @@
     {
         const char* e = LT_EXP_ENV("LT_TOPHAT_BRUTE");
         c->brute_tophat = e && e[0] == '1';
+    }
+    build_live_rows(*calib, warp, r0, r1 - r0, c->live_tasks.rows);
+    full_live_rows(calib->warp_h, calib->warp_w, c->full_tasks.rows);
+    {
+        const char* e = LT_EXP_ENV("LT_LIVE_TASKS");
+        c->live_tasks_on = !(e && e[0] == '0');
     }
 
     if (trace_on()) trace_line("lt_create:host_tables", t_tables);
@@ -1555,6 +1563,34 @@
     return LT_OK;
 }
 
+int lt_live_tasks(const lt_calib* calib, int k, int stage, int window, int cull, int band_rows, int32_t* tasks, int cap, int* n_tasks,
+                  int* n_pair, int32_t* strip_rows, double* dead_fraction) {
+    if (!calib || !n_tasks || !n_pair) return fail(LT_ERR_INVALID, "null argument");
+    if (k < 3 || k > 63 || !(k & 1) || stage < 0 || stage > 2 || window < 0 || cap < 0 || (cap > 0 && !tasks))
+        return fail(LT_ERR_INVALID, "lt_live_tasks: k odd in 3..63, stage 0..2, window >= 0");
+    if (calib->warp_w <= 0 || calib->warp_h <= 0) return fail(LT_ERR_INVALID, "lt_live_tasks: empty bird's-eye view");
+    LiveRows lr;
+    RemapTable warp;
+    build_warp_table(*calib, warp);
+    int r0 = 0, r1 = 0;
+    warp_source_rows(*calib, warp, r0, r1);
+    build_live_rows(*calib, warp, r0, r1 - r0, lr);
+    if (dead_fraction) *dead_fraction = lr.dead_fraction;
+    if (!cull) full_live_rows(calib->warp_h, calib->warp_w, lr);
+    const int h = calib->warp_h, w = calib->warp_w, R = k / 2;
+    const int margin = stage == 0 ? R : stage == 1 ? 2 * R : 2 * R + window;
+    const bool pair_strip = w % 4 == 0 && w - 128 * ((w + 127) / 128 - 1) <= 64;
+    std::vector<LiveTask> t;
+    std::vector<int32_t> sr;
+    int np = 0;
+    build_live_tasks(lr, margin, std::min(2 * R, h), band_rows > 0 ? band_rows : (h + 3) / 4, pair_strip, t, np, &sr);
+    *n_tasks = (int)t.size();
+    *n_pair = np;
+    for (int i = 0; i < (int)t.size() && i < cap; ++i) std::memcpy(tasks + 4 * (size_t)i, &t[(size_t)i], sizeof(LiveTask));
+    if (strip_rows) std::memcpy(strip_rows, sr.data(), sr.size() * sizeof(int32_t));
+    return LT_OK;
+}
+
 int lt_calib_lab_tables(uint16_t* gamma256, uint16_t* cbrt3072, int32_t* coeffs9) {
     if (!gamma256 || !cbrt3072 || !coeffs9) return fail(LT_ERR_INVALID, "null argument");
     build_lab_tables(gamma256, cbrt3072, coeffs9);
@@ -1839,7 +1875,9 @@
                                 ps, m); }
             for (int i = f0; i < f0 + m && i < (int)c->front_ok.size(); ++i) c->front_ok[(size_t)i] = 1;
         }
-        int frc = run_filter_chain(c, st, f0, m, p, c->calib.warp_h, c->calib.warp_w, n);
+        bool warped_here = f0 + m <= (int)c->front_ok.size();
+        for (int i = f0; warped_here && i < f0 + m; ++i) warped_here = c->front_ok[(size_t)i] != 0;
+        int frc = run_filter_chain(c, st, f0, m, p, c->calib.warp_h, c->calib.warp_w, n, false, warped_here);
         return frc ? frc : note_written_frame(c, st, f0, f0 + m, n);
     });
     if (rc) return rc;
diff --git a/lane_tracker_amd/csrc/lt_ctx.h b/lane_tracker_amd/csrc/lt_ctx.h
--- a/lane_tracker_amd/csrc/lt_ctx.h
+++ b/lane_tracker_amd/csrc/lt_ctx.h
@@ -91,6 +91,8 @@
     int maxpix = 0, maxlev = 0, maxbands = 0;
     bool have_mask = false;
     bool brute_tophat = false;
+    lt::LiveTaskCache live_tasks, full_tasks;
+    bool live_tasks_on = true;
     int16_t* d_oxy = nullptr;
     uint16_t* d_ofrac = nullptr;
     bool have_overlay = false;
diff --git a/lane_tracker_amd/csrc/lt_internal.h b/lane_tracker_amd/csrc/lt_internal.h
--- a/lane_tracker_amd/csrc/lt_internal.h
+++ b/lane_tracker_amd/csrc/lt_internal.h
@@ -30,6 +30,32 @@
 struct EllipseSE {
     int k;
     int8_t dx[64];
+};
+
+struct LiveRows {
+    int h = 0, w = 0;
+    std::vector<int32_t> lx0, lx1;
+    double dead_fraction = 0.0;
+};
+void build_live_rows(const lt_calib& c, const RemapTable& warp, int r0, int nrows, LiveRows& out);
+void full_live_rows(int h, int w, LiveRows& out);
+struct LiveTask {
+    int32_t strip, y0, rows, flags;
+};
+void build_live_tasks(const LiveRows& lr, int margin, int min_rows, int band_rows, bool pair_strip, std::vector<LiveTask>& tasks,
+                      int& n_pair, std::vector<int32_t>* strip_rows = nullptr);
+struct LiveTable {
+    int margin, min_rows, band_rows, pair_strip, n_pair, n_normal;
+    LiveTask* d_tasks;
+};
+struct LiveTaskCache {
+    LiveRows rows;
+    std::vector<LiveTable> tables;
+    LiveTaskCache() = default;
+    LiveTaskCache(const LiveTaskCache&) = delete;
+    LiveTaskCache& operator=(const LiveTaskCache&) = delete;
+    ~LiveTaskCache();
+    const LiveTable* get(int margin, int min_rows, int band_rows, bool pair_strip);
 };
 
 struct FrontEndGeom {
@@ -110,7 +136,8 @@
 void launch_morph_ellipse(hipStream_t s, const uint8_t* src, uint8_t* dst, const uint8_t* minuend, int h, int w,
                           const EllipseSE& se, bool dilate, size_t plane_stride, int n);
 bool launch_morph_runs(hipStream_t s, const uint8_t* src, uint8_t* dst, const uint8_t* minuend, int h, int w, int k,
-                       bool dilate, size_t plane_stride, int n, int dpitch = 0, size_t dst_stride = 0, uint8_t* copy_dst = nullptr);
+                       bool dilate, size_t plane_stride, int n, int dpitch = 0, size_t dst_stride = 0, uint8_t* copy_dst = nullptr,
+                       LiveTaskCache* live = nullptr);
 bool launch_morph_one_pair(hipStream_t s, const uint8_t* src55, uint8_t* dst55, const uint8_t* min55, const uint8_t* src29, uint8_t* dst29,
                            const uint8_t* min29, int h, int w, bool dilate, size_t plane_stride, int n, int dpitch, size_t dst_stride);
 bool tophat_tables_match(const EllipseSE& se29, const EllipseSE& se55);
diff --git a/lane_tracker_amd/csrc/lt_tables.cpp b/lane_tracker_amd/csrc/lt_tables.cpp
--- a/lane_tracker_amd/csrc/lt_tables.cpp
+++ b/lane_tracker_amd/csrc/lt_tables.cpp
@@ -1,3 +1,4 @@
+#include <algorithm>
 #include <cfloat>
 #include <climits>
 #include <cmath>
@@ -135,6 +136,106 @@
     }
 }
 
+void build_live_rows(const lt_calib& c, const RemapTable& warp, int r0, int nrows, LiveRows& out) {
+    out.h = warp.rows;
+    out.w = warp.cols;
+    out.lx0.assign((size_t)out.h, out.w);
+    out.lx1.assign((size_t)out.h, 0);
+    size_t dead = 0;
+    for (int y = 0; y < out.h; ++y)
+        for (int x = 0; x < out.w; ++x) {
+            const size_t o = (size_t)y * out.w + x;
+            const int sx = warp.xy[o * 2], sy = warp.xy[o * 2 + 1], ry0 = sy - r0, ry1 = ry0 + 1;
+            const bool y0 = sy >= 0 && sy < c.img_h && ry0 >= 0 && ry0 < nrows;
+            const bool y1 = sy + 1 >= 0 && sy + 1 < c.img_h && ry1 >= 0 && ry1 < nrows;
+            const bool x0 = sx >= 0 && sx < c.img_w, x1 = sx + 1 >= 0 && sx + 1 < c.img_w;
+            if ((y0 || y1) && (x0 || x1)) {
+                if (x < out.lx0[(size_t)y]) out.lx0[(size_t)y] = x;
+                out.lx1[(size_t)y] = x + 1;
+            } else
+                ++dead;
+        }
+    const size_t n = (size_t)out.h * out.w;
+    out.dead_fraction = n ? (double)dead / (double)n : 0.0;
+}
+
+void full_live_rows(int h, int w, LiveRows& out) {
+    out.h = h;
+    out.w = w;
+    out.lx0.assign((size_t)(h > 0 ? h : 0), 0);
+    out.lx1.assign((size_t)(h > 0 ? h : 0), w);
+    out.dead_fraction = 0.0;
+}
+
+void build_live_tasks(const LiveRows& lr, int margin, int min_rows, int band_rows, bool pair_strip, std::vector<LiveTask>& tasks,
+                      int& n_pair, std::vector<int32_t>* strip_rows) {
+    tasks.clear();
+    n_pair = 0;
+    if (strip_rows) strip_rows->clear();
+    const int h = lr.h, w = lr.w;
+    if (h <= 0 || w <= 0) return;
+    const int nstrips = (w + 127) / 128;
+    min_rows = std::min(std::max(min_rows, 1), h);
+    band_rows = std::max(band_rows, min_rows);
+    std::vector<LiveTask> normal, pair;
+    for (int strip = 0; strip < nstrips; ++strip) {
+        const int c0 = strip * 128 - margin, c1 = std::min(strip * 128 + 128, w) + margin;
+        int first = -1, last = -1;
+        for (int y = 0; y < h; ++y)
+            if (lr.lx0[(size_t)y] < lr.lx1[(size_t)y] && lr.lx1[(size_t)y] > c0 && lr.lx0[(size_t)y] < c1) {
+                if (first < 0) first = y;
+                last = y;
+            }
+        int ya = first < 0 ? 0 : std::max(first - margin, 0), yb = first < 0 ? 0 : std::min(last + 1 + margin, h);
+        if (yb - ya < min_rows) {
+            yb = std::min(ya + min_rows, h);
+            ya = std::max(yb - min_rows, 0);
+        }
+        if (strip_rows) { strip_rows->push_back(ya); strip_rows->push_back(yb); }
+        const int len = yb - ya;
+        int nb = std::max(1, (len + band_rows / 2) / band_rows);
+        while (nb > 1 && len / nb < min_rows) --nb;
+        const int base = len / nb, rem = len % nb;
+        std::vector<LiveTask>& dst = pair_strip && strip == nstrips - 1 ? pair : normal;
+        for (int b = 0, y = ya; b < nb; ++b) {
+            const int rows = base + (b < rem ? 1 : 0);
+            dst.push_back(LiveTask{strip, y, rows, (b == 0 && ya > 0 ? 1 : 0) | (b == nb - 1 && yb < h ? 2 : 0)});
+            y += rows;
+        }
+    }
+    auto longest_first = [](const LiveTask& a, const LiveTask& b) { return a.rows > b.rows; };
+    std::stable_sort(pair.begin(), pair.end(), longest_first);
+    std::stable_sort(normal.begin(), normal.end(), longest_first);
+    n_pair = (int)pair.size();
+    tasks = pair;
+    tasks.insert(tasks.end(), normal.begin(), normal.end());
+}
+
+LiveTaskCache::~LiveTaskCache() {
+    for (LiveTable& t : tables)
+        if (t.d_tasks) (void)hipFree(t.d_tasks);
+}
+
+const LiveTable* LiveTaskCache::get(int margin, int min_rows, int band_rows, bool pair_strip) {
+    for (const LiveTable& t : tables)
+        if (t.margin == margin && t.min_rows == min_rows && t.band_rows == band_rows && t.pair_strip == (pair_strip ? 1 : 0)) return &t;
+    constexpr size_t kMaxTables = 64;
+    if (tables.capacity() < kMaxTables) tables.reserve(kMaxTables);
+    if (tables.size() >= kMaxTables) return nullptr;
+    std::vector<LiveTask> tasks;
+    int n_pair = 0;
+    build_live_tasks(rows, margin, min_rows, band_rows, pair_strip, tasks, n_pair);
+    if (tasks.empty()) return nullptr;
+    LiveTable t{margin, min_rows, band_rows, pair_strip ? 1 : 0, n_pair, (int)tasks.size() - n_pair, nullptr};
+    if (hipMalloc(reinterpret_cast<void**>(&t.d_tasks), tasks.size() * sizeof(LiveTask)) != hipSuccess) return nullptr;
+    if (hipMemcpy(t.d_tasks, tasks.data(), tasks.size() * sizeof(LiveTask), hipMemcpyHostToDevice) != hipSuccess) {
+        (void)hipFree(t.d_tasks);
+        return nullptr;
+    }
+    tables.push_back(t);
+    return &tables.back();
+}
+
 void build_lab_tables(uint16_t gamma_tab[256], uint16_t cbrt_tab[3072], int32_t coeffs[9]) {
     auto to_u16 = [](float v) {
         int r = cv_round((double)v);
```

Measured after the change: 97440 frames/s. Within noise of the previous version (-0.9%).
